# Yotsuei/ClearConverse

Hardware: AMD Instinct MI355X
Metric: xRT (audio-sec/wall-sec) end-to-end, 30 s 16 kHz clips (higher is better)
Workload: dtype bf16

## Files before the change

### clearconverse_amd/_lib.py

```python
from __future__ import annotations

import ctypes as C
import os
from pathlib import Path
from typing import Optional

_PKG = Path(__file__).resolve().parent
LIB_PATH = _PKG / "libccx.so"


class CcxError(RuntimeError):
    pass


class WhisperDims(C.Structure):
    _fields_ = [(n, C.c_int) for n in (
        "n_mels", "n_audio_ctx", "n_audio_state", "n_audio_head", "n_audio_layer",
        "n_vocab", "n_text_ctx", "n_text_state", "n_text_head", "n_text_layer")]


class SepformerDims(C.Structure):
    _fields_ = [(n, C.c_int) for n in (
        "n_filters", "kernel", "stride", "d_model", "n_head", "d_ffn", "n_layers", "n_blocks", "segment", "n_spk")]


class DecodeRules(C.Structure):
    _fields_ = [(n, C.c_int) for n in (
        "eot", "sot", "sot_prev", "no_speech", "no_timestamps", "timestamp_begin", "blank",
        "max_initial_timestamp_index", "n_suppress")] + [("suppress", C.POINTER(C.c_int))]


class DecodeOptions(C.Structure):
    _fields_ = [("without_timestamps", C.c_int), ("suppress_blank", C.c_int), ("max_initial_timestamp_index", C.c_int),
                ("n_suppress", C.c_int), ("suppress", C.POINTER(C.c_int))]


class GemmDesc(C.Structure):
    _fields_ = [
        ("A", C.c_void_p), ("W", C.c_void_p), ("lda", C.c_int64), ("ldw", C.c_int64),
        ("M", C.c_int), ("N", C.c_int), ("K", C.c_int), ("ntaps", C.c_int), ("a_tap_stride", C.c_int64),
        ("bias", C.c_void_p), ("out", C.c_void_p), ("ldo", C.c_int64), ("resid", C.c_void_p), ("ldr", C.c_int64),
        ("resid_mod", C.c_int), ("scale", C.c_void_p), ("shift", C.c_void_p), ("slope", C.c_float),
        ("rpb_in", C.c_int), ("rpb_out", C.c_int), ("roff", C.c_int), ("rpb_valid", C.c_int),
        ("img_rows_in", C.c_int), ("img_rows_valid", C.c_int), ("img_rows_out", C.c_int),
        ("resid_bf16", C.c_void_p), ("ldrb", C.c_int64),
        ("hq", C.c_void_p), ("hk", C.c_void_p), ("hv", C.c_void_p),
        ("d_model", C.c_int), ("n_head", C.c_int), ("S", C.c_int), ("Spad", C.c_int),
        ("v_transposed", C.c_int), ("first_block", C.c_int),
        ("a_elems", C.c_int64), ("w_elems", C.c_int64), ("out_elems", C.c_int64), ("resid_elems", C.c_int64),
        ("resid_bf16_elems", C.c_int64), ("heads_elems", C.c_int64)]


class DecAttnDesc(C.Structure):
    _fields_ = [
        ("q", C.c_void_p), ("k", C.c_void_p), ("v", C.c_void_p),
        ("rows", C.c_int), ("n_seq", C.c_int), ("H", C.c_int), ("kv_T", C.c_int), ("T", C.c_int),
        ("pos", C.POINTER(C.c_int)), ("row_seq", C.POINTER(C.c_int)), ("rows_per_seq", C.c_int),
        ("nsplit", C.c_int), ("combine", C.c_int), ("lds_pad", C.c_int),
        ("x", C.c_void_p), ("pend", C.c_void_p), ("pend_n", C.c_int), ("pend_stride", C.c_int64),
        ("ln_g", C.c_void_p), ("ln_b", C.c_void_p), ("eps", C.c_float),
        ("wq_host", C.c_void_p), ("bq", C.c_void_p),
        ("out", C.c_void_p), ("part_o", C.c_void_p), ("part_ml", C.c_void_p), ("q_x_out", C.c_void_p),
        ("q_elems", C.c_int64), ("kv_elems", C.c_int64), ("out_elems", C.c_int64), ("part_o_elems", C.c_int64),
        ("part_ml_elems", C.c_int64), ("x_elems", C.c_int64), ("pend_elems", C.c_int64), ("q_x_out_elems", C.c_int64),
        ("ind", C.POINTER(C.c_uint16)), ("ind_ld", C.c_int)]


DEC_ATTN_SELF, DEC_ATTN_SPLIT, DEC_ATTN_STREAM, DEC_ATTN_PREFILL, DEC_ATTN_FUSED_Q, DEC_ATTN_TWO_LAUNCH_Q = range(6)
DEC_ATTN_STREAM_MAPPED = 7
DEC_ATTN_SELF_IND = 8


class DecLnLinearDesc(C.Structure):
    _fields_ = [
        ("M", C.c_int), ("K", C.c_int), ("F", C.c_int), ("N", C.c_int), ("epi", C.c_int), ("packed", C.c_int),
        ("x", C.c_void_p), ("ln_g", C.c_void_p), ("ln_b", C.c_void_p), ("eps", C.c_float),
        ("w1_host", C.c_void_p), ("b1", C.c_void_p), ("w_host", C.c_void_p), ("bias", C.c_void_p),
        ("out", C.c_void_p), ("x_elems", C.c_int64), ("out_elems", C.c_int64)]


class DecodeSamplingOptions(C.Structure):
    _fields_ = [("top_k", C.c_int), ("top_p", C.c_float), ("min_p", C.c_float)]


class DecSeqState(C.Structure):
    _fields_ = [(n, C.c_int) for n in ("pos", "prompt_len", "n_gen", "done", "last_tok", "pen_tok", "last_ts_tok", "n_tokens")] + [
        ("sum_logprob", C.c_float), ("no_speech_prob", C.c_float)]


class DecSelectDesc(C.Structure):
    _fields_ = [
        ("logits", C.c_void_p), ("ld", C.c_int64), ("n_vocab", C.c_int), ("B", C.c_int),
        ("rules", C.POINTER(DecodeRules)), ("state", C.POINTER(DecSeqState)),
        ("prompt", C.POINTER(C.c_int)), ("max_prompt", C.c_int), ("sample_len", C.c_int),
        ("gen", C.POINTER(C.c_int)), ("cur_tok", C.POINTER(C.c_int)), ("pos", C.POINTER(C.c_int)), ("n_done", C.POINTER(C.c_int)),
        ("tok_emb", C.c_void_p), ("pos_emb", C.c_void_p), ("x", C.c_void_p), ("D", C.c_int),
        ("sample", C.c_int), ("temperature", C.c_float), ("seed", C.c_uint64), ("row0", C.c_int),
        ("logits_elems", C.c_int64), ("tok_emb_elems", C.c_int64), ("pos_emb_elems", C.c_int64), ("x_elems", C.c_int64),
        ("stream_ids", C.POINTER(C.c_int)), ("opts", C.POINTER(DecodeOptions)),
        ("sampling", C.POINTER(DecodeSamplingOptions)), ("cut_out", C.POINTER(C.c_float)), ("kept_out", C.POINTER(C.c_int)),
        ("kept_mass_out", C.POINTER(C.c_float))]


class DecBeamDesc(C.Structure):
    _fields_ = [
        ("logits", C.c_void_p), ("ld", C.c_int64), ("n_vocab", C.c_int),
        ("G", C.c_int), ("beam_size", C.c_int), ("max_candidates", C.c_int),
        ("rules", C.POINTER(DecodeRules)), ("state", C.POINTER(DecSeqState)), ("sample_len", C.c_int),
        ("hist", C.POINTER(C.c_int)), ("cur_tok", C.POINTER(C.c_int)), ("pos", C.POINTER(C.c_int)), ("n_done", C.POINTER(C.c_int)),
        ("tok_emb", C.c_void_p), ("pos_emb", C.c_void_p), ("x", C.c_void_p), ("D", C.c_int),
        ("ind", C.POINTER(C.c_uint16)), ("ind_ld", C.c_int),
        ("fin_tok", C.POINTER(C.c_int)), ("fin_score", C.POINTER(C.c_float)), ("fin_n", C.POINTER(C.c_int)),
        ("fin_count", C.POINTER(C.c_int)),
        ("cand_id", C.POINTER(C.c_int)), ("cand_lp", C.POINTER(C.c_float)), ("tok_out", C.POINTER(C.c_int)),
        ("parent_out", C.POINTER(C.c_int)),
        ("logits_elems", C.c_int64), ("tok_emb_elems", C.c_int64), ("pos_emb_elems", C.c_int64), ("x_elems", C.c_int64),
        ("opts", C.POINTER(DecodeOptions))]


class DecodeHistoryOptions(C.Structure):
    _fields_ = [("repetition_penalty", C.c_float), ("no_repeat_ngram_size", C.c_int)]


# ... 141 lines not shown
_ip = C.POINTER(C.c_int)
_i32p = C.POINTER(C.c_int32)
_i64p = C.POINTER(C.c_int64)
_fp = C.POINTER(C.c_float)

PROTOTYPES = {
    "ccx_version": (C.c_char_p, []),
    "ccx_ctx_create": (_i, [_i, C.POINTER(_vp)]),
    "ccx_ctx_destroy": (None, [_vp]),
    "ccx_last_error": (C.c_char_p, [_vp]),
    "ccx_prof_enable": (_i, [_vp, _i]),
    "ccx_prof_count": (_i, [_vp]),
    "ccx_prof_get": (_i, [_vp, _i, C.c_char_p, _i, C.POINTER(C.c_double), C.POINTER(C.c_double), _fp]),
    "ccx_gemm_bf16": (_i, [_vp, _i, _vp, _i64, _vp, _i64, _vp, _vp, _i64, _vp, _i64, _i, _i, _i, _vp]),
    "ccx_gemm_bf16_desc": (_i, [_vp, _i, C.POINTER(GemmDesc), _vp]),
    "ccx_layernorm": (_i, [_vp, _vp, _vp, _vp, _vp, _vp, _i, _i, _f, _vp]),
    "ccx_gather_rows": (_i, [_vp, _vp, _vp, _i, _i, _vp, _i64, _vp]),
    "ccx_peak_normalize": (_i, [_vp, _vp, _vp, _i64, _vp, _i, _f, _vp]),
    "ccx_row_variance": (_i, [_vp, _vp, _i64, _vp, _i, _vp, _vp]),
    "ccx_cross_attention_xa": (_i, [_vp, _vp, _vp, _vp, _vp, _vp, _vp, _i, _i, _i, _i, _i, _vp, _vp]),
    "ccx_cosine_rows": (_i, [_vp, _vp, _vp, _i, _i, _i, _vp, _vp]),
    "ccx_speaker_profiles": (_i, [_vp, _vp, _vp, _vp, _i, _i, _i, _i, _vp, _vp]),
    "ccx_resample_sinc": (_i, [_vp, _vp, _i64, _vp, _i, _i, _i, _i, _vp, _vp, _i64, _vp, _i, _vp]),
    "ccx_enc_attention": (_i, [_vp, _vp, _vp, _vp, _vp, _i, _i, _i, _i, _vp]),
    "ccx_whisper_create": (_i, [_vp, C.POINTER(WhisperDims), _i, C.POINTER(_vp)]),
    "ccx_whisper_destroy": (None, [_vp]),
    "ccx_whisper_set_tensor": (_i, [_vp, C.c_char_p, _vp, _i, _i, _i64p]),
    "ccx_whisper_set_max_audio": (_i, [_vp, C.c_double]),
    "ccx_whisper_share_encoder_scratch": (_i, [_vp, _vp]),
    "ccx_whisper_finalize": (_i, [_vp]),
    "ccx_whisper_set_rules": (_i, [_vp, C.POINTER(DecodeRules)]),
    "ccx_whisper_logmel": (_i, [_vp, _vp, _i64, _ip, _ip, _i, _vp, _vp]),
    "ccx_whisper_logmel_ex": (_i, [_vp, _vp, _i64, _ip, _ip, _ip, _i, _vp, _vp]),
    "ccx_decode_options_default": (None, [C.POINTER(DecodeOptions)]),
    "ccx_whisper_set_decode_options": (_i, [_vp, C.POINTER(DecodeOptions)]),
    "ccx_whisper_graph_count": (_i, [_vp, _i]),
    "ccx_decode_history_options_default": (None, [C.POINTER(DecodeHistoryOptions)]),
    "ccx_whisper_set_history_options": (_i, [_vp, C.POINTER(DecodeHistoryOptions)]),
    "ccx_whisper_history_graph_count": (_i, [_vp]),
    "ccx_dec_history_step": (_i, [_vp, C.POINTER(DecHistoryDesc), _vp]),
    "ccx_decode_bias_options_default": (None, [C.POINTER(DecodeBiasOptions)]),
    "ccx_whisper_set_bias_options": (_i, [_vp, C.POINTER(DecodeBiasOptions)]),
    "ccx_whisper_bias_graph_count": (_i, [_vp]),
    "ccx_dec_bias_step": (_i, [_vp, C.POINTER(DecBiasDesc), _vp]),
    "ccx_decode_sampling_options_default": (None, [C.POINTER(DecodeSamplingOptions)]),
    "ccx_whisper_set_sampling_options": (_i, [_vp, C.POINTER(DecodeSamplingOptions)]),
    "ccx_whisper_sampling_graph_count": (_i, [_vp]),
    "ccx_whisper_set_mel": (_i, [_vp, _vp, _i, _vp]),
    "ccx_whisper_encode": (_i, [_vp, _i, _vp, _vp]),
    "ccx_whisper_decoder_logits": (_i, [_vp, _i32p, _i, _i, _vp, _vp]),
    "ccx_whisper_decode_greedy": (_i, [_vp, _i32p, _i32p, _i, _i, _i, _i32p, _i32p, _fp, _fp, _vp]),
    "ccx_dec_attention_desc": (_i, [_vp, _i, C.POINTER(DecAttnDesc), _vp]),
    "ccx_dec_ln_linear": (_i, [_vp, C.POINTER(DecLnLinearDesc), _vp]),
    "ccx_dec_select_step": (_i, [_vp, C.POINTER(DecSelectDesc), _vp]),
    "ccx_dec_beam_step": (_i, [_vp, C.POINTER(DecBeamDesc), _vp]),
    "ccx_whisper_decode_beam": (_i, [_vp, _i32p, _i32p, _i, _i, _i32p, _i, _i, _i, _i, _i32p, _i32p, _fp, _i32p, _fp,
                                     C.POINTER(BeamTrace), _vp]),
    "ccx_dec_token_probs": (_i, [_vp, C.POINTER(DecTokenProbsDesc), _vp]),
    "ccx_dec_pick_probs": (_i, [_vp, C.POINTER(DecPickProbsDesc), _vp]),
    "ccx_align_op": (_i, [_vp, _i, C.POINTER(AlignDesc), _vp]),
    "ccx_whisper_align": (_i, [_vp, _i32p, _i32p, _i, _i, _i32p, _i32p, _i, _i, _vp, _vp, _i32p, _vp]),
    "ccx_whisper_align_probs": (_i, [_vp, _i32p, _i32p, _i, _i, _i32p, _i32p, _i, _i, _vp, _vp, _i32p, _i, _fp, _vp]),
    "ccx_whisper_last_cross_path": (_i, [_vp]),
    "ccx_whisper_set_sot_tail": (_i, [_vp, _i]),
    "ccx_whisper_set_prefix_len": (_i, [_vp, _i]),
    "ccx_whisper_detect_language": (_i, [_vp, _i, _i, _i, _i32p, _fp, _vp]),
    "ccx_whisper_prepare_lanes": (_i, [_vp, _vp]),
    "ccx_whisper_trace_lanes": (_i, [_vp, C.c_char_p, _i]),
    "ccx_whisper_decode": (_i, [_vp, _i32p, _i32p, _i, _i, _i, _f, C.c_uint64, _i32p, _i32p, _fp, _fp, _vp]),
    "ccx_whisper_decode_rows": (_i, [_vp, _i32p, _i32p, _i, _i, _i32p, _i, _i32p, _i, _f, C.c_uint64, _i32p, _i32p, _fp, _fp, _vp]),
    "ccx_sepformer_create": (_i, [_vp, C.POINTER(SepformerDims), _i, _i, C.POINTER(_vp)]),
    "ccx_sepformer_destroy": (None, [_vp]),
    "ccx_sepformer_set_tensor": (_i, [_vp, C.c_char_p, _vp, _i64]),
    "ccx_sepformer_finalize": (_i, [_vp]),
    "ccx_sepformer_separate": (_i, [_vp, _vp, _i64, _ip, _i, _vp, _vp]),
    "ccx_sep_op": (_i, [_vp, _i, C.POINTER(SepDesc), _vp]),
    "ccx_speaker_create": (_i, [_vp, _i, _i, _i, _i, _i64, C.POINTER(_vp)]),
    "ccx_speaker_destroy": (None, [_vp]),
    "ccx_speaker_set_tensor": (_i, [_vp, C.c_char_p, _vp, _i64]),
    "ccx_speaker_finalize": (_i, [_vp]),
    "ccx_speaker_embed": (_i, [_vp, _vp, _i64p, _ip, _i, _vp, _i64p, _ip, _vp, _vp]),
    "ccx_speaker_segment": (_i, [_vp, _vp, _i64p, _ip, _i, _vp, _i64, _ip, _vp]),
    "ccx_speaker_op": (_i, [_vp, _i, C.POINTER(SpeakerDesc), _vp]),
    "ccx_ecapa_create": (_i, [_vp, _i, _i64, C.POINTER(_vp)]),
    "ccx_ecapa_destroy": (None, [_vp]),
    "ccx_ecapa_set_tensor": (_i, [_vp, C.c_char_p, _vp, _i64]),
    "ccx_ecapa_finalize": (_i, [_vp]),
    "ccx_ecapa_embed": (_i, [_vp, _vp, _i64p, _ip, _i, _vp, _vp]),
    "ccx_ecapa_op": (_i, [_vp, _i, C.POINTER(EcapaDesc), _vp]),
    "ccx_resnet_create": (_i, [_vp, _i, _i64, _i, C.POINTER(_vp)]),
    "ccx_resnet_destroy": (None, [_vp]),
    "ccx_resnet_set_tensor": (_i, [_vp, C.c_char_p, _vp, _i64]),
    "ccx_resnet_finalize": (_i, [_vp]),
    "ccx_resnet_embed": (_i, [_vp, _vp, _i64, _i, _i, _vp, _i, _ip, _i, _vp, _vp]),
    "ccx_resnet_op": (_i, [_vp, _i, C.POINTER(ResnetDesc), _vp]),
    "ccx_specgate_create": (_i, [_vp, _i64, _i, _i, C.POINTER(_vp)]),
    "ccx_specgate_destroy": (None, [_vp]),
    "ccx_specgate_reduce": (_i, [_vp, _vp, _i64, _ip, _i, _f, _vp, _vp]),
    "ccx_specgate_reduce_long": (_i, [_vp, _vp, _i64, _f, _vp, _vp]),
    "ccx_specgate_set_clip_noise": (_i, [_vp, _i]),
    "ccx_specgate_opts_default": (None, [C.POINTER(SpecgateOpts)]),
    "ccx_specgate_reduce_ex": (_i, [_vp, C.POINTER(SpecgateOpts), _vp, _i64, _ip, _i, _vp, _vp]),
    "ccx_specgate_reduce_long_ex": (_i, [_vp, C.POINTER(SpecgateOpts), _vp, _i64, _vp, _vp]),
    "ccx_specgate_time_smooth": (_i, [_vp, _vp, _vp, _ip, _i, _i64, _f, _vp]),
}

# ... 80 lines not shown
```

### clearconverse_amd/csrc/cross_x.h

```cpp
#pragma once
#include "ccx_common.h"

struct XsParams {
  const float* q;
  const float* x; const float* pend; int pend_n; long pend_stride;
  float* x_out;
  const float* ln_g; const float* ln_b; float eps;
  const bf16_t* Wq;
  const float* bq;
  const bf16_t* xb; const float2* ln_stats; const float* ln_s;
  const bf16_t* WkT;
  bf16_t* xq;
  float* part_o;
  float* part_ml;
  const bf16_t* X;
  long x_seq_stride;
  const int* row_seq;
  int rows_per_seq;
  const bf16_t* Wv;
  const float* bv;
  bf16_t* out;
  int rows, H, S, D;
  float scale_log2e;
  int lds_pad;
  int full_lines;
};

int ccx_xs_full_lines_switch();

#define XS_SPLIT 2
static inline size_t ccx_xs_part_o_elems(size_t rows, int H, int D) { return rows * XS_SPLIT * (size_t)H * D; }
static inline size_t ccx_xs_part_ml_elems(size_t rows) { return rows * XS_SPLIT * 16 * 2; }
int ccx_launch_xs_cross_attention(ccx_ctx* ctx, const XsParams& p, hipStream_t stream);
bool ccx_xs_supported(int D, int H);
```

### clearconverse_amd/csrc/cross_x.hip

```cpp
#include "cross_x.h"
#include "dec_ln.h"

namespace {

typedef __attribute__((ext_vector_type(4))) uint32_t u32x4;
typedef __attribute__((ext_vector_type(2))) uint32_t u32x2;

__device__ __forceinline__ bf16x8 pack8(const float4 a, const float4 b) {
  const u32x4 v = {pack_bf16x2(a.x, a.y), pack_bf16x2(a.z, a.w), pack_bf16x2(b.x, b.y), pack_bf16x2(b.z, b.w)};
  return __builtin_bit_cast(bf16x8, v);
}

}

template <int D>
__global__ __launch_bounds__(256) void dec_xq_expand_kernel(XsParams p) {
  constexpr int FW = D / 4, NMT = FW / 16;
  const int h = blockIdx.x, r0 = blockIdx.y * 16;
  const int wave = threadIdx.x >> 6, lane = threadIdx.x & 63, n = lane & 15, g = lane >> 4;
  int row = r0 + n;
  const bool live = row < p.rows;
  if (!live) row = p.rows - 1;
  bf16x8 qb[2];
#pragma unroll
  for (int ks = 0; ks < 2; ks++) {
    const float4* src = (const float4*)(p.q + (long)row * D + h * 64 + ks * 32 + g * 8);
    qb[ks] = pack8(src[0], src[1]);
  }
  const bf16_t* wbase = p.WkT + ((long)h * D + wave * FW + n) * 64 + g * 8;
  bf16_t* dst = p.xq + ((long)row * p.H + h) * D + wave * FW + g * 4;
#pragma unroll
  for (int mt = 0; mt < NMT; mt++) {
    const bf16x8 a0 = *(const bf16x8*)(wbase + (long)mt * 16 * 64);
    const bf16x8 a1 = *(const bf16x8*)(wbase + (long)mt * 16 * 64 + 32);
    f32x4 c = {0.f, 0.f, 0.f, 0.f};
    c = __builtin_amdgcn_mfma_f32_16x16x32_bf16(a0, qb[0], c, 0, 0, 0);
    c = __builtin_amdgcn_mfma_f32_16x16x32_bf16(a1, qb[1], c, 0, 0, 0);
    if (live) *(u32x2*)(dst + mt * 16) = (u32x2){pack_bf16x2(c[0], c[1]), pack_bf16x2(c[2], c[3])};
  }
}

__device__ __forceinline__ float xs_wave_sum(float v) { return wave_reduce_sum(v); }

template <int D>
__global__ __launch_bounds__(256) void dec_xq_fused_kernel(XsParams p) {
  constexpr int NKS = D / 32, FW = D / 4, NMT = FW / 16, RSX = 2 * D + 16, RSQ = 2 * 64 + 16, NV = D / 4, NI = (NV + 63) / 64;
  __shared__ __attribute__((aligned(16))) char xn_s[16 * RSX];
  __shared__ __attribute__((aligned(16))) char q_s[16 * RSQ];
  const int h = blockIdx.x, r0 = blockIdx.y * 16;
  const int wave = threadIdx.x >> 6, lane = threadIdx.x & 63, n = lane & 15, g = lane >> 4;
  bf16x8 wq[NKS];
  {
    const bf16_t* wsrc = p.Wq + (long)(h * 64 + wave * 16 + n) * D + g * 8;
#pragma unroll
    for (int ks = 0; ks < NKS; ks++) wq[ks] = *(const bf16x8*)(wsrc + ks * 32);
  }
  {
    float4 gg[NI], bb[NI];
#pragma unroll
    for (int i = 0; i < NI; i++) {
      const int idx = lane + 64 * i, ic = idx < NV ? idx : 0;
      gg[i] = ((const float4*)p.ln_g)[ic];
      bb[i] = ((const float4*)p.ln_b)[ic];
    }
#pragma unroll
    for (int rr = 0; rr < 4; rr++) {
      const int lr = wave * 4 + rr;
      int m = r0 + lr;
      const bool live = m < p.rows;
      if (!live) m = p.rows - 1;
      float4 v[NI];
      float sm = 0.f;
#pragma unroll
      for (int i = 0; i < NI; i++) {
        const int idx = lane + 64 * i, ic = idx < NV ? idx : 0;
        float4 a = ((const float4*)(p.x + (long)m * D))[ic];
        float4 q[4];
#pragma unroll
        for (int s2 = 0; s2 < 4; s2++) q[s2] = ((const float4*)(p.pend + (long)(s2 < p.pend_n ? s2 : 0) * p.pend_stride + (long)m * D))[ic];
#pragma unroll
        for (int s2 = 0; s2 < 4; s2++) a = ln_add_pend(a, s2 < p.pend_n ? 1.f : 0.f, q[s2]);
        if (idx >= NV) a = make_float4(0.f, 0.f, 0.f, 0.f);
        v[i] = a;
        if (p.x_out && h == 0 && live && idx < NV) ((float4*)(p.x_out + (long)m * D))[idx] = a;
        sm += ln_sum4(a);
      }
      const float mean = xs_wave_sum(sm) / (float)D;
      float sq = 0.f;
#pragma unroll
      for (int i = 0; i < NI; i++) {
        const float t = ln_sq4(v[i], mean);
        sq += (lane + 64 * i < NV) ? t : 0.f;
      }
      const float rstd = rsqrtf(xs_wave_sum(sq) / (float)D + p.eps);
#pragma unroll
      for (int i = 0; i < NI; i++) {
        const int idx = lane + 64 * i;
        if (idx < NV) *(uint2*)(xn_s + lr * RSX + idx * 8) = ln_pack4(v[i], mean, rstd, gg[i], bb[i]);
      }
    }
  }
  __syncthreads();
  f32x4 ca = {0.f, 0.f, 0.f, 0.f}, cb = {0.f, 0.f, 0.f, 0.f};
  {
    const char* xsrc = xn_s + n * RSX + g * 16;
#pragma unroll
    for (int ks = 0; ks < NKS; ks++) {
      const bf16x8 b = *(const bf16x8*)(xsrc + ks * 64);
      if (ks & 1) cb = __builtin_amdgcn_mfma_f32_16x16x32_bf16(wq[ks], b, cb, 0, 0, 0);
      else ca = __builtin_amdgcn_mfma_f32_16x16x32_bf16(wq[ks], b, ca, 0, 0, 0);
    }
  }
  const bf16_t* wbase = p.WkT + ((long)h * D + wave * FW + n) * 64 + g * 8;
  bf16x8 wk[NMT][2];
#pragma unroll
  for (int mt = 0; mt < NMT; mt++) {
    wk[mt][0] = *(const bf16x8*)(wbase + (long)mt * 16 * 64);
    wk[mt][1] = *(const bf16x8*)(wbase + (long)mt * 16 * 64 + 32);
  }
  {
    const float4 bias = *(const float4*)(p.bq + h * 64 + wave * 16 + g * 4);
    const float v0 = ca[0] + cb[0] + bias.x, v1 = ca[1] + cb[1] + bias.y, v2 = ca[2] + cb[2] + bias.z, v3 = ca[3] + cb[3] + bias.w;
    *(u32x2*)(q_s + n * RSQ + (wave * 16 + g * 4) * 2) = (u32x2){pack_bf16x2(v0, v1), pack_bf16x2(v2, v3)};
  }
  __syncthreads();
  const bf16x8 qb0 = *(const bf16x8*)(q_s + n * RSQ + g * 16), qb1 = *(const bf16x8*)(q_s + n * RSQ + 64 + g * 16);
  const int row = r0 + n;
  bf16_t* dst = p.xq + ((long)(row < p.rows ? row : p.rows - 1) * p.H + h) * D + wave * FW + g * 4;
#pragma unroll
  for (int mt = 0; mt < NMT; mt++) {
    f32x4 c = {0.f, 0.f, 0.f, 0.f};
    c = __builtin_amdgcn_mfma_f32_16x16x32_bf16(wk[mt][0], qb0, c, 0, 0, 0);
    c = __builtin_amdgcn_mfma_f32_16x16x32_bf16(wk[mt][1], qb1, c, 0, 0, 0);
    if (row < p.rows) *(u32x2*)(dst + mt * 16) = (u32x2){pack_bf16x2(c[0], c[1]), pack_bf16x2(c[2], c[3])};
  }
}

template <int D>
__global__ __launch_bounds__(256) void dec_xq_lnfree_kernel(XsParams p) {
  constexpr int NKS = D / 32, FW = D / 4, NMT = FW / 16, RSQ = 2 * 64 + 16;
  __shared__ __attribute__((aligned(16))) char q_s[16 * RSQ];
  __shared__ float2 st_s[16];
  const int h = blockIdx.x, r0 = blockIdx.y * 16;
  const int wave = threadIdx.x >> 6, lane = threadIdx.x & 63, n = lane & 15, g = lane >> 4;
  int row = r0 + n;
  const bool live = row < p.rows;
  if (!live) row = p.rows - 1;
  bf16x8 wq[NKS], xb[NKS];
  {
    const bf16_t* wsrc = p.Wq + (long)(h * 64 + wave * 16 + n) * D + g * 8;
    const bf16_t* xsrc = p.xb + (long)row * D + g * 8;
#pragma unroll
    for (int ks = 0; ks < NKS; ks++) wq[ks] = *(const bf16x8*)(wsrc + ks * 32);
#pragma unroll
    for (int ks = 0; ks < NKS; ks++) xb[ks] = *(const bf16x8*)(xsrc + ks * 32);
  }
  if (threadIdx.x < 64) {
    const int r = threadIdx.x >> 2, qt = threadIdx.x & 3;
    int m = r0 + r;
    m = m < p.rows ? m : p.rows - 1;
    constexpr int T4 = (D / 16) / 4;
    const float2* sp = p.ln_stats + (long)m * (D / 16) + qt * T4;
    float s1 = 0.f, s2 = 0.f;
#pragma unroll
    for (int i = 0; i < T4; i++) {
      const float2 v = sp[i];
      s1 += v.x; s2 += v.y;
    }
    s1 += dpp_mov<CCX_DPP_QUAD_XOR1>(s1); s2 += dpp_mov<CCX_DPP_QUAD_XOR1>(s2);
    s1 += dpp_mov<CCX_DPP_QUAD_XOR2>(s1); s2 += dpp_mov<CCX_DPP_QUAD_XOR2>(s2);
    const float mean = s1 / (float)D;
    const float var = fmaf(-mean, mean, s2 / (float)D);
    if (qt == 0) st_s[r] = make_float2(mean, rsqrtf(fmaxf(var, 0.f) + p.eps));
  }
  const bf16_t* wbase = p.WkT + ((long)h * D + wave * FW + n) * 64 + g * 8;
  bf16x8 wk[NMT][2];
#pragma unroll
  for (int mt = 0; mt < NMT; mt++) {
    wk[mt][0] = *(const bf16x8*)(wbase + (long)mt * 16 * 64);
    wk[mt][1] = *(const bf16x8*)(wbase + (long)mt * 16 * 64 + 32);
  }
  const float4 cc = *(const float4*)(p.bq + h * 64 + wave * 16 + g * 4);
  const float4 ss = *(const float4*)(p.ln_s + h * 64 + wave * 16 + g * 4);
  f32x4 ca = {0.f, 0.f, 0.f, 0.f}, cb = {0.f, 0.f, 0.f, 0.f};
#pragma unroll
  for (int ks = 0; ks < NKS; ks++) {
    if (ks & 1) cb = __builtin_amdgcn_mfma_f32_16x16x32_bf16(wq[ks], xb[ks], cb, 0, 0, 0);
    else ca = __builtin_amdgcn_mfma_f32_16x16x32_bf16(wq[ks], xb[ks], ca, 0, 0, 0);
  }
  __syncthreads();
  {
    const float2 ms = st_s[n];
    const float v0 = fmaf(ms.y, fmaf(-ms.x, ss.x, ca[0] + cb[0]), cc.x), v1 = fmaf(ms.y, fmaf(-ms.x, ss.y, ca[1] + cb[1]), cc.y);
    const float v2 = fmaf(ms.y, fmaf(-ms.x, ss.z, ca[2] + cb[2]), cc.z), v3 = fmaf(ms.y, fmaf(-ms.x, ss.w, ca[3] + cb[3]), cc.w);
    *(u32x2*)(q_s + n * RSQ + (wave * 16 + g * 4) * 2) = (u32x2){pack_bf16x2(v0, v1), pack_bf16x2(v2, v3)};
  }
  __syncthreads();
  const bf16x8 qb0 = *(const bf16x8*)(q_s + n * RSQ + g * 16), qb1 = *(const bf16x8*)(q_s + n * RSQ + 64 + g * 16);
  bf16_t* dst = p.xq + ((long)row * p.H + h) * D + wave * FW + g * 4;
#pragma unroll
  for (int mt = 0; mt < NMT; mt++) {
    f32x4 c = {0.f, 0.f, 0.f, 0.f};
    c = __builtin_amdgcn_mfma_f32_16x16x32_bf16(wk[mt][0], qb0, c, 0, 0, 0);
    c = __builtin_amdgcn_mfma_f32_16x16x32_bf16(wk[mt][1], qb1, c, 0, 0, 0);
    if (live) *(u32x2*)(dst + mt * 16) = (u32x2){pack_bf16x2(c[0], c[1]), pack_bf16x2(c[2], c[3])};
  }
}

template <int D>
__global__ __launch_bounds__(256) void dec_xv_project_kernel(XsParams p) {
  constexpr int NKS = D / 32, RSB = 2 * D + 16;
  __shared__ __attribute__((aligned(16))) char ctx_s[16 * RSB];
  const int h = blockIdx.x, r0 = blockIdx.y * 16;
  const int wave = threadIdx.x >> 6, lane = threadIdx.x & 63, n = lane & 15, g = lane >> 4;
  const int o0 = h * 64 + wave * 16;
  const bf16_t* wsrc = p.Wv + (long)(o0 + n) * D + g * 8;
  constexpr int CH = NKS % 6 == 0 ? 6 : 4;
  static_assert(NKS % CH == 0, "D must be a multiple of 128");
  bf16x8 a[CH];
#pragma unroll
  for (int k = 0; k < CH; k++) a[k] = *(const bf16x8*)(wsrc + k * 32);
  {
    const int rr = threadIdx.x >> 4, c = threadIdx.x & 15;
    int row = r0 + rr;
    if (row >= p.rows) row = p.rows - 1;
    float m[XS_SPLIT], l[XS_SPLIT], wgt[XS_SPLIT];
    float mx = -INFINITY;
#pragma unroll
    for (int s2 = 0; s2 < XS_SPLIT; s2++) {
      const float2 ml = *(const float2*)(p.part_ml + (((long)row * XS_SPLIT + s2) * 16 + h) * 2);
      m[s2] = ml.x; l[s2] = ml.y;
      mx = fmaxf(mx, ml.x);
    }
    float den = 0.f;
#pragma unroll
    for (int s2 = 0; s2 < XS_SPLIT; s2++) {
      wgt[s2] = __builtin_amdgcn_exp2f(m[s2] - mx);
      den = fmaf(l[s2], wgt[s2], den);
    }
    const float inv = 1.f / den;
#pragma unroll
    for (int s2 = 0; s2 < XS_SPLIT; s2++) wgt[s2] *= inv;
    const float* src = p.part_o + (((long)row * XS_SPLIT) * p.H + h) * D;
    const long sstride = (long)p.H * D;
#pragma unroll
    for (int k = 0; k < D / 64; k++) {
      const int f = (c + 16 * k) * 4;
      float4 v = make_float4(0.f, 0.f, 0.f, 0.f);
#pragma unroll
      for (int s2 = 0; s2 < XS_SPLIT; s2++) {
        const float4 o = *(const float4*)(src + s2 * sstride + f);
        v.x = fmaf(o.x, wgt[s2], v.x); v.y = fmaf(o.y, wgt[s2], v.y); v.z = fmaf(o.z, wgt[s2], v.z); v.w = fmaf(o.w, wgt[s2], v.w);
      }
      *(u32x2*)(ctx_s + rr * RSB + f * 2) = (u32x2){pack_bf16x2(v.x, v.y), pack_bf16x2(v.z, v.w)};
    }
  }
  __syncthreads();
  const char* csrc = ctx_s + n * RSB + g * 16;
  f32x4 ca = {0.f, 0.f, 0.f, 0.f}, cb = {0.f, 0.f, 0.f, 0.f};
#pragma unroll
  for (int c0 = 0; c0 < NKS; c0 += CH) {
    bf16x8 an[CH];
    if (c0 + CH < NKS) {
#pragma unroll
      for (int k = 0; k < CH; k++) an[k] = *(const bf16x8*)(wsrc + (c0 + CH + k) * 32);
    }
#pragma unroll
    for (int k = 0; k < CH; k++) {
      const bf16x8 b = *(const bf16x8*)(csrc + (c0 + k) * 64);
      if (k & 1) cb = __builtin_amdgcn_mfma_f32_16x16x32_bf16(a[k], b, cb, 0, 0, 0);
      else ca = __builtin_amdgcn_mfma_f32_16x16x32_bf16(a[k], b, ca, 0, 0, 0);
    }
    if (c0 + CH < NKS) {
#pragma unroll
      for (int k = 0; k < CH; k++) a[k] = an[k];
    }
  }
  const int row = r0 + n;
  if (row < p.rows) {
    const float4 bias = *(const float4*)(p.bv + o0 + g * 4);
    const float v0 = ca[0] + cb[0] + bias.x, v1 = ca[1] + cb[1] + bias.y, v2 = ca[2] + cb[2] + bias.z, v3 = ca[3] + cb[3] + bias.w;
    *(u32x2*)(p.out + (long)row * D + o0 + g * 4) = (u32x2){pack_bf16x2(v0, v1), pack_bf16x2(v2, v3)};
  }
}

namespace {
#ifndef CCX_XS_FULL_NT
#define CCX_XS_FULL_NT 1
#endif
template <int D, int RB = 1, int FL = 0>
struct XsGeom {
  static constexpr int FW = D / 4;
  static constexpr int NKS = FW / 32;
  static constexpr int NMT = FW / 16;
  static constexpr int PF = 4;
  static constexpr int RS = 2 * FW + 32;
  static constexpr int STRIP = 16 * RS;
  static constexpr int NSTRIP = FL ? 2 : 1;
  static constexpr int S_OFF = 4 * NSTRIP * STRIP;
  static constexpr int LDS = S_OFF + 2 * RB * 4 * 1024;
  static_assert(!FL || (D / 2) % 128 == 0, "full lines: a wave's quarter of a key row must be whole 128-byte lines");
  static_assert(!FL || PF % 2 == 0, "full lines: the strip of a tile is the parity of its slot");
};
template <int D> constexpr bool xs_full_lines_ok = (D / 2) % 128 == 0;
}

template <int D, int RB, int FL>
__global__ __launch_bounds__(256, RB == 1 ? 2 : 1) void dec_xs_stream_kernel(XsParams p) {
  using G = XsGeom<D, RB, FL>;
  constexpr int FW = G::FW, NKS = G::NKS, NMT = G::NMT, PF = G::PF, RS = G::RS, STRIP = G::STRIP;
  constexpr bool FULL = FL != 0, NT_HINT = CCX_XS_FULL_NT != 0;
  extern __shared__ __attribute__((aligned(16))) char xs_smem[];
  const int unit = blockIdx.x / XS_SPLIT, sp = blockIdx.x % XS_SPLIT;
  int row0, nrow;
  if (RB == 1) { row0 = unit; nrow = 1; }
  else {
    const int groups = (p.rows_per_seq + RB - 1) / RB;
    const int s_idx = unit / groups, gi = unit - s_idx * groups;
    row0 = s_idx * p.rows_per_seq + gi * RB;
    nrow = p.rows_per_seq - gi * RB < RB ? p.rows_per_seq - gi * RB : RB;
  }
  const int seq = p.row_seq ? p.row_seq[row0] : row0;
  const int wave = threadIdx.x >> 6, lane = threadIdx.x & 63, r = lane & 15, g = lane >> 4;
  const int H = p.H, S = p.S;
  char* strip = xs_smem + wave * (G::NSTRIP * STRIP);
  char* sbuf = xs_smem + G::S_OFF;

  const int lk = FULL ? lane >> 3 : r, lc = FULL ? lane & 7 : g;
  const bf16_t* Xp = p.X + (long)seq * p.x_seq_stride + wave * FW + lc * 8;
  const int NTall = (S + 15) >> 4;
  const int T0 = NTall * sp / XS_SPLIT, NT = NTall * (sp + 1) / XS_SPLIT;

  bf16x8 img[PF][NKS];
  auto load_tile = [&](bf16x8 (&X)[NKS], int t) {
    int key = t * 16 + lk;
// ... 187 lines not shown
  CCX_REQUIRE(ctx, p.rows_per_seq <= 1 || p.row_seq != nullptr, "xs cross attention: rows_per_seq = %d needs row_seq", p.rows_per_seq);
  const bool multi = p.rows_per_seq > 1;
  CCX_REQUIRE(ctx, p.rows_per_seq <= 1 || p.rows % p.rows_per_seq == 0, "xs cross attention: %d rows are not a multiple of %d rows per sequence", p.rows, p.rows_per_seq);
  const dim3 small_grid(p.H, ccx_cdiv(p.rows, 16));
  const double wbytes = (double)p.H * 64 * D * 2;
  if (p.xb) {
    ccx_prof_scope ps(ctx, stream, D == 768 ? "dec_xq_lnfree_kernel<768>" : "dec_xq_lnfree_kernel", 2.0 * p.rows * D * (double)D * 2,
                      2.0 * wbytes + (double)p.rows * D * 2 + (double)p.rows * p.H * D * 2);
    hipLaunchKernelGGL(dec_xq_lnfree_kernel<D>, small_grid, dim3(256), 0, stream, p);
  } else if (p.x) {
    ccx_prof_scope ps(ctx, stream, D == 768 ? "dec_xq_fused_kernel<768>" : "dec_xq_fused_kernel", 2.0 * p.rows * D * (double)D * 2,
                      2.0 * wbytes + (double)p.rows * D * 4 * (1 + p.pend_n) + (double)p.rows * p.H * D * 2);
    hipLaunchKernelGGL(dec_xq_fused_kernel<D>, small_grid, dim3(256), 0, stream, p);
  } else {
    ccx_prof_scope ps(ctx, stream, D == 768 ? "dec_xq_expand_kernel<768>" : "dec_xq_expand_kernel", 2.0 * p.rows * p.H * 64 * D, wbytes + (double)p.rows * D * 4 + (double)p.rows * p.H * D * 2);
    hipLaunchKernelGGL(dec_xq_expand_kernel<D>, small_grid, dim3(256), 0, stream, p);
  }
  CCX_CHECK_LAUNCH(ctx);
  {
    ccx_prof_scope ps(ctx, stream, D == 768 ? (multi ? "dec_xs_stream_kernel<768,4>" : "dec_xs_stream_kernel<768,1>") : "dec_xs_stream_kernel", 4.0 * p.rows * 16 * (double)p.S * D,
                      (double)p.rows * ((double)p.S * D * 2 + p.H * D * 2.0 + XS_SPLIT * p.H * D * 4.0));
    int rc;
    if constexpr (xs_full_lines_ok<D>) {
      rc = p.full_lines ? launch_xs_stream<D, 1>(ctx, p, stream) : launch_xs_stream<D, 0>(ctx, p, stream);
    } else {
      rc = launch_xs_stream<D, 0>(ctx, p, stream);
    }
    if (rc != CCX_OK) return rc;
  }
  CCX_CHECK_LAUNCH(ctx);
  {
    ccx_prof_scope ps(ctx, stream, D == 768 ? "dec_xv_project_kernel<768>" : "dec_xv_project_kernel", 2.0 * p.rows * p.H * 64 * D, wbytes + (double)p.rows * p.H * D * 2 + (double)p.rows * D * 2);
    hipLaunchKernelGGL(dec_xv_project_kernel<D>, small_grid, dim3(256), 0, stream, p);
  }
  CCX_CHECK_LAUNCH(ctx);
  return CCX_OK;
}

}

int ccx_xs_full_lines_switch() {
  const char* e = getenv("CCX_XS_FULL_LINES");
  return !e || atoi(e) != 0;
}

bool ccx_xs_supported(int D, int H) { return H >= 1 && H <= 16 && H * 64 == D && (D == 128 || D == 256 || D == 384 || D == 512 || D == 768); }

int ccx_launch_xs_cross_attention(ccx_ctx* ctx, const XsParams& p, hipStream_t stream) {
  CCX_REQUIRE(ctx, ccx_xs_supported(p.D, p.H), "xs cross attention: width %d with %d heads is not instantiated", p.D, p.H);
  CCX_REQUIRE(ctx, p.rows >= 1 && p.S >= 16 && (p.q || p.x || p.xb) && p.WkT && p.xq && p.X && p.Wv && p.bv && p.out, "xs cross attention: bad arguments");
  CCX_REQUIRE(ctx, !p.xb || (p.ln_stats && p.ln_s && p.Wq && p.bq), "xs cross attention: bad LayerNorm-free query arguments");
  CCX_REQUIRE(ctx, !p.x || (p.pend && p.ln_g && p.ln_b && p.Wq && p.bq && p.pend_n >= 0 && p.pend_n <= 4 && p.x_out != p.x), "xs cross attention: bad fused-query arguments");
  CCX_REQUIRE(ctx, p.part_o && p.part_ml, "xs cross attention: partial buffers missing");
  switch (p.D) {
    case 128: return launch_xs<128>(ctx, p, stream);
    case 256: return launch_xs<256>(ctx, p, stream);
    case 384: return launch_xs<384>(ctx, p, stream);
    case 512: return launch_xs<512>(ctx, p, stream);
    default: return launch_xs<768>(ctx, p, stream);
  }
}

namespace {
__global__ void xs_bf16_to_f32_kernel(const bf16_t* __restrict__ in, float* __restrict__ out, long n) {
  const long i = (long)blockIdx.x * 256 + threadIdx.x;
  if (i < n) out[i] = bf16_to_f32(in[i]);
}
}

extern "C" int ccx_cross_attention_xa(ccx_ctx* ctx, const float* q_dev, const float* wk_host, const float* wv_host, const float* bv_host,
                                      const uint16_t* xa_dev, const int* row_seq_host, int rows_per_seq, int rows, int n_seq, int n_head,
                                      int n_ctx, float* out_dev, void* stream_) {
  if (!ctx) return CCX_ERR_ARG;
  hipStream_t stream = (hipStream_t)stream_;
  const int H = n_head, D = 64 * n_head, S = n_ctx;
  CCX_REQUIRE(ctx, ccx_xs_supported(D, H), "cross_attention_xa: %d heads (width %d) not instantiated", H, D);
  CCX_REQUIRE(ctx, q_dev && wk_host && wv_host && bv_host && xa_dev && out_dev && rows >= 1 && n_seq >= 1 && S >= 16, "cross_attention_xa: bad arguments");
  if (row_seq_host)
    for (int i = 0; i < rows; i++) CCX_REQUIRE(ctx, row_seq_host[i] >= 0 && row_seq_host[i] < n_seq, "cross_attention_xa: row_seq[%d] out of range", i);
  else CCX_REQUIRE(ctx, rows <= n_seq, "cross_attention_xa: more rows than sequences without a row map");
  if (rows_per_seq > 1) {
    CCX_REQUIRE(ctx, row_seq_host && rows % rows_per_seq == 0, "cross_attention_xa: rows_per_seq needs a row map and a multiple of it in rows");
    for (int i = 0; i < rows; i++)
      CCX_REQUIRE(ctx, row_seq_host[i] == row_seq_host[i - i % rows_per_seq], "cross_attention_xa: row %d is not in its group's sequence", i);
  }
  std::vector<bf16_t> wkt((size_t)D * D), wv((size_t)D * D);
  for (int hh = 0; hh < H; hh++)
    for (int f = 0; f < D; f++)
      for (int dd = 0; dd < 64; dd++) wkt[((size_t)hh * D + f) * 64 + dd] = ccx_host_f32_to_bf16(wk_host[(size_t)(hh * 64 + dd) * D + f]);
  for (size_t i = 0; i < wv.size(); i++) wv[i] = ccx_host_f32_to_bf16(wv_host[i]);
  bf16_t *d_wkt = nullptr, *d_wv = nullptr, *d_xq = nullptr, *d_out = nullptr;
  float *d_bv = nullptr, *d_po = nullptr, *d_pml = nullptr;
  int* d_rs = nullptr;
  auto cleanup = [&]() { hipFree(d_wkt); hipFree(d_wv); hipFree(d_xq); hipFree(d_out); hipFree(d_bv); hipFree(d_rs); hipFree(d_po); hipFree(d_pml); };
#define XS_TRY(expr) do { hipError_t e_ = (expr); if (e_ != hipSuccess) { cleanup(); return ccx_fail(ctx, CCX_ERR_HIP, "%s failed: %s", #expr, hipGetErrorString(e_)); } } while (0)
  XS_TRY(hipMalloc(&d_wkt, wkt.size() * 2)); XS_TRY(hipMalloc(&d_wv, wv.size() * 2)); XS_TRY(hipMalloc(&d_bv, (size_t)D * 4));
  XS_TRY(hipMalloc(&d_xq, (size_t)rows * H * D * 2)); XS_TRY(hipMalloc(&d_out, (size_t)rows * D * 2));
  XS_TRY(hipMalloc(&d_po, ccx_xs_part_o_elems(rows, H, D) * 4)); XS_TRY(hipMalloc(&d_pml, ccx_xs_part_ml_elems(rows) * 4));
  XS_TRY(hipMemcpy(d_wkt, wkt.data(), wkt.size() * 2, hipMemcpyHostToDevice));
  XS_TRY(hipMemcpy(d_wv, wv.data(), wv.size() * 2, hipMemcpyHostToDevice));
  XS_TRY(hipMemcpy(d_bv, bv_host, (size_t)D * 4, hipMemcpyHostToDevice));
  if (row_seq_host) {
    XS_TRY(hipMalloc(&d_rs, (size_t)rows * 4));
    XS_TRY(hipMemcpy(d_rs, row_seq_host, (size_t)rows * 4, hipMemcpyHostToDevice));
  }
  XsParams p;
  memset(&p, 0, sizeof(p));
  p.q = q_dev; p.WkT = d_wkt; p.xq = d_xq; p.X = xa_dev; p.x_seq_stride = (long)S * D; p.row_seq = d_rs; p.Wv = d_wv; p.bv = d_bv; p.out = d_out; p.part_o = d_po; p.part_ml = d_pml;
  p.rows = rows; p.H = H; p.S = S; p.D = D; p.scale_log2e = 0.125f * 1.4426950408889634f;
  p.rows_per_seq = rows_per_seq > 1 ? rows_per_seq : 0;
  p.full_lines = ccx_xs_full_lines_switch();
  int rc =ccx_launch_xs_cross_attention(ctx, p, stream);
  if (rc == CCX_OK) {
    const long n = (long)rows * D;
    hipLaunchKernelGGL(xs_bf16_to_f32_kernel, dim3((unsigned)((n + 255) / 256)), dim3(256), 0, stream, d_out, out_dev, n);
    XS_TRY(hipStreamSynchronize(stream));
  }
  cleanup();
#undef XS_TRY
  return rc;
}
```

### clearconverse_amd/csrc/dec_ops.hip

```cpp
#include "../../include/ccx.h"
#include "ccx_common.h"
#include "decoder.h"
#include "op_scratch.h"

static_assert(sizeof(ccx_dec_seq_state) == sizeof(DecSeqState), "ccx_dec_seq_state mirrors DecSeqState field for field");

namespace {

__global__ void dec_ops_bf16_to_f32_kernel(const bf16_t* __restrict__ in, float* __restrict__ out, long n) {
  const long i = (long)blockIdx.x * 256 + threadIdx.x;
  if (i < n) out[i] = bf16_to_f32(in[i]);
}

}

extern "C" int ccx_dec_attention_desc(ccx_ctx* ctx, int form, const ccx_dec_attn_desc* d, void* stream_) {
  if (!ctx) return CCX_ERR_ARG;
  hipStream_t stream = (hipStream_t)stream_;
  CCX_REQUIRE(ctx, d != nullptr, "ccx_dec_attention_desc: desc is NULL");
  CCX_REQUIRE(ctx, (form >= CCX_DEC_ATTN_SELF && form <= CCX_DEC_ATTN_TWO_LAUNCH_Q) || form == CCX_DEC_ATTN_STREAM_MAPPED || form == CCX_DEC_ATTN_SELF_IND,
              "ccx_dec_attention_desc: unknown form %d", form);
  const bool is_ind = form == CCX_DEC_ATTN_SELF_IND;
  const bool is_self = form == CCX_DEC_ATTN_SELF || is_ind, is_split = form == CCX_DEC_ATTN_SPLIT, is_mapped = form == CCX_DEC_ATTN_STREAM_MAPPED,
             is_stream = form == CCX_DEC_ATTN_STREAM || is_mapped;
  const bool is_prefill = form == CCX_DEC_ATTN_PREFILL, with_q = form == CCX_DEC_ATTN_FUSED_Q || form == CCX_DEC_ATTN_TWO_LAUNCH_Q;
  const bool partials = is_split || with_q;
  const bool final_out = is_self || is_stream || is_prefill || (is_split && d->combine);
  const int rows = d->rows, H = d->H, n_seq = d->n_seq, kv_T = d->kv_T;
  CCX_REQUIRE(ctx, rows >= 1 && rows <= 65536 && n_seq >= 1 && n_seq <= 65536 && H >= 1 && H <= 64 && kv_T >= 1 && kv_T <= (1 << 20),
              "ccx_dec_attention_desc: rows=%d, n_seq=%d, H=%d or kv_T=%d out of range", rows, n_seq, H, kv_T);
  CCX_REQUIRE(ctx, d->k && d->v && ccx_aligned16(d->k) && ccx_aligned16(d->v), "ccx_dec_attention_desc: k / v null or not 16-byte aligned");
  const int64_t kv_need = (int64_t)n_seq * H * kv_T * 64;
  CCX_REQUIRE(ctx, kv_need <= d->kv_elems, "ccx_dec_attention_desc: k / v are read up to element %ld, kv_elems=%ld", (long)kv_need, (long)d->kv_elems);
  if (is_ind) {
    CCX_REQUIRE(ctx, d->row_seq == nullptr, "ccx_dec_attention_desc: row_seq is not taken by form %d (the rows read through ind)", form);
  } else if (is_self || is_split || is_prefill || is_mapped) {
    if (d->row_seq)
      for (int i = 0; i < rows; i++)
        CCX_REQUIRE(ctx, d->row_seq[i] >= 0 && d->row_seq[i] < n_seq, "ccx_dec_attention_desc: row_seq[%d] = %d out of range [0, %d)", i, d->row_seq[i], n_seq);
    else CCX_REQUIRE(ctx, rows <= n_seq, "ccx_dec_attention_desc: row_seq is NULL with more rows (%d) than sequences (%d)", rows, n_seq);
  } else {
    CCX_REQUIRE(ctx, d->row_seq == nullptr, "ccx_dec_attention_desc: row_seq is not taken by form %d (row r reads sequence r)", form);
    CCX_REQUIRE(ctx, rows <= n_seq, "ccx_dec_attention_desc: more rows (%d) than sequences (%d)", rows, n_seq);
  }
  if (is_prefill) {
    const int P = d->rows_per_seq;
    CCX_REQUIRE(ctx, P >= 2 && P <= 4096, "ccx_dec_attention_desc: rows_per_seq = %d, the prefill form needs >= 2", P);
    CCX_REQUIRE(ctx, d->row_seq && rows % P == 0, "ccx_dec_attention_desc: rows_per_seq needs row_seq and a multiple of it in rows");
    for (int i = 0; i < rows; i++) {
      CCX_REQUIRE(ctx, d->row_seq[i] == d->row_seq[i - i % P], "ccx_dec_attention_desc: row %d is not in its group's sequence (row_seq)", i);
      CCX_REQUIRE(ctx, d->row_seq[i] == i / P, "ccx_dec_attention_desc: row_seq[%d] = %d, the prefill form needs group g on sequence g", i, d->row_seq[i]);
    }
  } else CCX_REQUIRE(ctx, d->rows_per_seq <= 1, "ccx_dec_attention_desc: rows_per_seq = %d is taken by the prefill form only", d->rows_per_seq);
  if (is_self) {
    CCX_REQUIRE(ctx, d->pos != nullptr, "ccx_dec_attention_desc: pos is NULL");
// ... 148 lines not shown
  bf16_t *d_xn = nullptr, *d_ffn = nullptr, *d_w1 = nullptr, *d_w = nullptr, *d_g16 = nullptr, *d_ck = nullptr, *d_cv = nullptr;
  float* d_pend = nullptr; int* d_pos = nullptr;
  DO_HIP(sc.alloc(&d_xn, Mp * K));
  DO_HIP(hipMemsetAsync(d_xn, 0xFF, Mp * K * 2, stream));
  DO_HIP(sc.alloc(&d_pend, (size_t)M * K));
  DO_HIP(hipMemsetAsync(d_pend, 0, (size_t)M * K * 4, stream));
  DO_HIP(hipMemsetAsync(d->out, 0xFF, (size_t)n_out * 4, stream));
  {
    const std::vector<bf16_t> pw = pack_mfma_rows(d->w_host, N, Kin, 32);
    DO_HIP(sc.upload(&d_w, pw.data(), pw.size()));
  }
  int rc = ccx_launch_dec_resolve_ln(ctx, (const float*)d->x, d_pend, 0, (long)M * K, (const float*)d->ln_g, (const float*)d->ln_b, d_xn, nullptr, M, K,
                                     d->eps, stream, nullptr, packed);
  const bf16_t* act = d_xn;
  if (rc == CCX_OK && F > 0) {
    const std::vector<bf16_t> pw1 = pack_mfma_rows(d->w1_host, F, K, 32);
    DO_HIP(sc.upload(&d_w1, pw1.data(), pw1.size()));
    DO_HIP(sc.alloc(&d_ffn, Mp * F));
    DO_HIP(hipMemsetAsync(d_ffn, 0xFF, Mp * F * 2, stream));
    DecLinearParams lp;
    memset(&lp, 0, sizeof(lp));
    lp.M = M; lp.N = F; lp.K = K; lp.W = d_w1; lp.ldw = K; lp.bias = (const float*)d->b1; lp.act = d_xn; lp.lda = K; lp.act_packed = packed;
    lp.out = d_ffn; lp.ldo = F; lp.out_packed = packed;
    rc = ccx_launch_dec_linear(ctx, ACT_BF16, DEPI_BF16_GELU, lp, stream);
    act = d_ffn;
  }
  if (rc == CCX_OK) {
    DecLinearParams lp;
    memset(&lp, 0, sizeof(lp));
    lp.M = M; lp.N = N; lp.K = Kin; lp.W = d_w; lp.ldw = Kin; lp.bias = (const float*)d->bias; lp.act = act; lp.lda = Kin; lp.act_packed = packed;
    lp.out = d->out; lp.ldo = N; lp.pend_stride = (long)M * N;
    if (epi == CCX_DEC_EPI_SELF_QKV) {
      const std::vector<int> pos((size_t)M, 0);
      DO_HIP(sc.upload(&d_pos, pos.data(), pos.size()));
      DO_HIP(sc.alloc(&d_ck, (size_t)M * K)); DO_HIP(sc.alloc(&d_cv, (size_t)M * K));
      DO_HIP(hipMemsetAsync(d_ck, 0xFF, (size_t)M * K * 2, stream)); DO_HIP(hipMemsetAsync(d_cv, 0xFF, (size_t)M * K * 2, stream));
      lp.ldo = K; lp.cache_k = d_ck; lp.cache_v = d_cv; lp.cache_T = 1; lp.pos = d_pos;
    } else if (epi == CCX_DEC_EPI_GELU) {
      DO_HIP(sc.alloc(&d_g16, Mp * N));
      DO_HIP(hipMemsetAsync(d_g16, 0xFF, Mp * N * 2, stream));
      lp.out = d_g16; lp.out_packed = packed;
    }
    rc = ccx_launch_dec_linear(ctx, ACT_BF16, depi, lp, stream);
    if (rc == CCX_OK && epi == CCX_DEC_EPI_SELF_QKV) {
      const long n = (long)M * K;
      hipLaunchKernelGGL(dec_ops_rows_to_f32_kernel, dim3((unsigned)((n + 255) / 256)), dim3(256), 0, stream, d_ck, (float*)d->out + n, M, K, 0);
      hipLaunchKernelGGL(dec_ops_rows_to_f32_kernel, dim3((unsigned)((n + 255) / 256)), dim3(256), 0, stream, d_cv, (float*)d->out + 2 * n, M, K, 0);
      DO_HIP(hipGetLastError());
    } else if (rc == CCX_OK && epi == CCX_DEC_EPI_GELU) {
      const long n = (long)M * N;
      hipLaunchKernelGGL(dec_ops_rows_to_f32_kernel, dim3((unsigned)((n + 255) / 256)), dim3(256), 0, stream, d_g16, (float*)d->out, M, N, packed);
      DO_HIP(hipGetLastError());
    }
  }
  DO_HIP(hipStreamSynchronize(stream));
  return rc;
}

extern "C" int ccx_dec_select_step(ccx_ctx* ctx, const ccx_dec_select_desc* d, void* stream_) {
  if (!ctx) return CCX_ERR_ARG;
  hipStream_t stream = (hipStream_t)stream_;
  CCX_REQUIRE(ctx, d != nullptr, "ccx_dec_select_step: desc is NULL");
  const int V = d->n_vocab, B = d->B, D = d->D;
  CCX_REQUIRE(ctx, B >= 1 && B <= 65536, "ccx_dec_select_step: B = %d out of range", B);
  CCX_REQUIRE(ctx, V >= 4 && V % 4 == 0 && V <= 13 * 4096, "ccx_dec_select_step: n_vocab = %d must be a multiple of 4 and <= 53248", V);
  CCX_REQUIRE(ctx, d->ld >= V && d->ld % 4 == 0, "ccx_dec_select_step: ld = %ld must be >= n_vocab and a multiple of 4", (long)d->ld);
  CCX_REQUIRE(ctx, d->logits && ccx_aligned16(d->logits), "ccx_dec_select_step: logits null or not 16-byte aligned");
  CCX_REQUIRE(ctx, (int64_t)(B - 1) * d->ld + V <= d->logits_elems, "ccx_dec_select_step: logits are read up to element %ld, logits_elems=%ld",
              (long)((int64_t)(B - 1) * d->ld + V), (long)d->logits_elems);
  CCX_REQUIRE(ctx, d->rules && d->state && d->gen && d->cur_tok && d->pos && d->n_done, "ccx_dec_select_step: rules, state, gen, cur_tok, pos or n_done is NULL");
  const ccx_decode_rules& r = *d->rules;
  std::vector<unsigned char> mask;
  CCX_TRY(ccx_build_suppress_mask(ctx, "ccx_dec_select_step", &r, V, mask));
  int max_init_ts = r.max_initial_timestamp_index, no_rules = 0, sup_blank = 1;
  if (const ccx_decode_options* o = d->opts) {
    CCX_TRY(ccx_build_options_mask(ctx, "ccx_dec_select_step", &r, o, V, mask));
    no_rules = o->without_timestamps; sup_blank = o->suppress_blank;
    if (o->max_initial_timestamp_index != -2) max_init_ts = o->max_initial_timestamp_index;
  }
  CCX_REQUIRE(ctx, r.no_speech >= 0 && r.timestamp_begin >= 0 && r.blank >= 0, "ccx_dec_select_step: rules.no_speech, timestamp_begin or blank negative");
  CCX_REQUIRE(ctx, d->sample_len >= 1 && d->sample_len <= (1 << 20), "ccx_dec_select_step: sample_len = %d out of range", d->sample_len);
  CCX_REQUIRE(ctx, d->max_prompt >= 0 && (d->max_prompt == 0 || d->prompt), "ccx_dec_select_step: prompt is NULL with max_prompt = %d", d->max_prompt);
  CCX_REQUIRE(ctx, D >= 4 && D % 4 == 0 && D <= 4096, "ccx_dec_select_step: D = %d must be a multiple of 4 in [4, 4096]", D);
  CCX_REQUIRE(ctx, d->tok_emb && d->pos_emb && d->x && ccx_aligned16(d->tok_emb) && ccx_aligned16(d->pos_emb) && ccx_aligned16(d->x),
              "ccx_dec_select_step: tok_emb, pos_emb or x null or not 16-byte aligned");
  CCX_REQUIRE(ctx, (int64_t)V * D <= d->tok_emb_elems, "ccx_dec_select_step: tok_emb is read up to element %ld, tok_emb_elems=%ld", (long)V * D, (long)d->tok_emb_elems);
  CCX_REQUIRE(ctx, (int64_t)B * D <= d->x_elems, "ccx_dec_select_step: x is written up to element %ld, x_elems=%ld", (long)B * D, (long)d->x_elems);
  const int64_t pos_rows = d->pos_emb_elems / D;
  CCX_REQUIRE(ctx, d->sample == 0 || d->sample == 1, "ccx_dec_select_step: sample = %d must be 0 or 1", d->sample);
  CCX_REQUIRE(ctx, d->sample || d->temperature == 0.f, "ccx_dec_select_step: temperature %g needs sample = 1", (double)d->temperature);
  CCX_REQUIRE(ctx, d->temperature >= 0.f && d->row0 >= 0, "ccx_dec_select_step: temperature or row0 negative");
  ccx_decode_sampling_options trunc{0, 1.0f, 0.0f};
  if (d->sampling) {
    CCX_REQUIRE(ctx, d->sample == 1, "ccx_dec_select_step: sampling options need sample = 1");
    trunc = *d->sampling;
    CCX_TRY(ccx_check_sampling_options(ctx, "ccx_dec_select_step", &trunc));
  }
  CCX_REQUIRE(ctx, d->sampling || (!d->cut_out && !d->kept_out && !d->kept_mass_out), "ccx_dec_select_step: cut_out, kept_out and kept_mass_out need sampling options");
  if (d->stream_ids)
    for (int b = 0; b < B; b++) CCX_REQUIRE(ctx, d->stream_ids[b] >= 0, "ccx_dec_select_step: stream_ids[%d] = %d is negative", b, d->stream_ids[b]);
  for (int b = 0; b < B; b++) {
    const ccx_dec_seq_state& s = d->state[b];
    CCX_REQUIRE(ctx, s.n_gen >= 0 && s.n_gen <= d->sample_len, "ccx_dec_select_step: state[%d].n_gen = %d out of range [0, sample_len = %d]", b, s.n_gen, d->sample_len);
    CCX_REQUIRE(ctx, s.pos >= 0 && s.pos + 1 < pos_rows, "ccx_dec_select_step: state[%d].pos = %d, pos + 1 must be a row of pos_emb (%ld rows)", b, s.pos, (long)pos_rows);
    CCX_REQUIRE(ctx, s.prompt_len >= 0 && s.prompt_len <= d->max_prompt, "ccx_dec_select_step: state[%d].prompt_len = %d out of range [0, max_prompt = %d]", b, s.prompt_len, d->max_prompt);
    CCX_REQUIRE(ctx, s.done == 0 || s.done == 1, "ccx_dec_select_step: state[%d].done = %d must be 0 or 1", b, s.done);
// ... 188 lines not shown
```

### clearconverse_amd/csrc/decoder.h

```cpp
#pragma once
#include <cstring>
#include <vector>
#include "../../include/ccx.h"
#include "ccx_common.h"

enum { ACT_LN = 0, ACT_BF16 = 1, ACT_COMBINE = 2 };
enum { DEPI_BF16_GELU = 1, DEPI_PARTIAL = 2, DEPI_F32 = 3, DEPI_SELF_QKV = 4, DEPI_RESOLVE = 5 };

struct DecLinearParams {
  int M, N, K;
  const bf16_t* W; long ldw;
  const float* bias;
  const float* x;
  const float* pend; int pend_n; long pend_stride;
  float* x_out;
  const float* ln_g; const float* ln_b; float eps;
  float* ln_mean_out;
  const bf16_t* act; long lda;
  const float* part_o; const float* part_ml; int nsplit;
  float* xres; bf16_t* xb; float2* st_out; const float* shift; float shift_c;
  void* out; long ldo;
  bf16_t* cache_k; bf16_t* cache_v; int cache_T; const int* pos; const int* row_seq;
  int act_packed, out_packed;
};
int ccx_launch_dec_linear(ccx_ctx* ctx, int act, int epi, const DecLinearParams& p, hipStream_t stream);
int ccx_dec_linear_ksplit(int K, int epi);
int ccx_launch_dec_resolve_ln(ccx_ctx* ctx, const float* x, const float* pend, int pend_n, long pend_stride, const float* g,
                              const float* b, bf16_t* out, float* x_out, int M, int K, float eps, hipStream_t stream,
                              float* mean_out = nullptr, int out_packed = 0);

__host__ __device__ __forceinline__ long dec_frag_off(int m, int k, int ksteps) {
  return (((long)(m >> 4) * ksteps + (k >> 5)) * 64 + (((k >> 3) & 3) * 16 + (m & 15))) * 8 + (k & 7);
}
int ccx_dec_packed_act_switch();

struct DecAttnParams {
  const float* q;
  const bf16_t* k;
  const bf16_t* v;
  int H, kv_T;
  const int* pos;
  int T;
  float scale_log2e;
  bf16_t* out_bf16;
  float* part_o;
  float* part_ml;
  int lds_pad;
  int stream_mode;
  const int* row_seq; int rows_per_seq;
  const float* qx; const float* q_pend; int q_pend_n; long q_pend_stride; float* q_x_out;
  const float* q_ln_g; const float* q_ln_b; float q_eps;
  const bf16_t* q_W; const float* q_bias; int q_K;
  int kv_map;
  const unsigned short* ind; int ind_ld;
};
int ccx_launch_dec_attention(ccx_ctx* ctx, const DecAttnParams& p, int B, int nsplit, bool final_out, hipStream_t stream);
int ccx_launch_dec_cross_fused_q(ccx_ctx* ctx, const DecAttnParams& p, int B, int nsplit, hipStream_t stream);

struct DecSeqState {
  int pos, prompt_len, n_gen, done;
  int last_tok, pen_tok, last_ts_tok, n_tokens;
  float sum_logprob, no_speech_prob;
};

struct DecSelectParams {
  const float* logits; long ld_logits; int n_vocab;
  DecSeqState* state;
  const int* prompt; int max_prompt;
  int* cur_tok; int* pos;
  int* gen; int sample_len;
  int* n_done;
  const unsigned char* suppress_mask;
  int eot, blank, no_speech, timestamp_begin, max_initial_ts;
  const float* tok_emb; const float* pos_emb; float* x; int D;
  const unsigned* sample_cfg; int row0;
  int sample;
  const int* stream_id;
  int no_rules, suppress_blank;
  int trunc;
  float* cut_out; int* kept_out; float* kept_mass_out;
};
int ccx_launch_dec_select(ccx_ctx* ctx, const DecSelectParams& p, int B, hipStream_t stream);

constexpr int kBeamMax = 8;
constexpr int kBeamCandMax = 16;
struct DecBeamParams {
  DecSelectParams sel;
  int beam, max_cand;
  int* cand_id; float* cand_lp;
  unsigned short* ind; int ind_ld;
  int row0;
  int* fin_tok; float* fin_score; int* fin_n; int* fin_count;
  int* step_tok; int* step_parent;
  int* tr_cand_id; float* tr_cand_lp; int* tr_tok; int* tr_parent; float* tr_score; int tr_rows;
};
int ccx_launch_dec_beam(ccx_ctx* ctx, const DecBeamParams& p, int n_windows, hipStream_t stream);

constexpr int kDecHistoryMax = 2048;
struct DecHistoryParams {
  float* logits; long ld;
  const DecSeqState* state;
  const int* gen; int sample_len;
  int text_end;
  float penalty; int ngram;
};
int ccx_launch_dec_history(ccx_ctx* ctx, const DecHistoryParams& p, int rows, hipStream_t stream);

// ... 114 lines not shown
```

### clearconverse_amd/csrc/decoder.hip

```cpp
#include <string>
#include "decoder.h"

__global__ void dec_embed_kernel(const float* __restrict__ tok_emb, const float* __restrict__ pos_emb,
                                 const int* __restrict__ cur_tok, const int* __restrict__ pos, float* __restrict__ x,
                                 int D) {
  const int b = blockIdx.x;
  const float4* te = (const float4*)(tok_emb + (long)cur_tok[b] * D);
  const float4* pe = (const float4*)(pos_emb + (long)pos[b] * D);
  float4* xo = (float4*)(x + (long)b * D);
  for (int i = threadIdx.x; i < D / 4; i += blockDim.x) {
    const float4 a = te[i], c = pe[i];
    xo[i] = make_float4(a.x + c.x, a.y + c.y, a.z + c.z, a.w + c.w);
  }
}

#include "dec_ln.h"

__device__ __forceinline__ float centre_shift(float mean, float rstd) { return fabsf(mean) * rstd > 1.f ? mean : 0.f; }

__device__ __forceinline__ uint4 combine_partials(const float* part_o, const float* part_ml, int nsplit, int mh, int c) {
  const float2* ml = (const float2*)(part_ml + ((long)mh * nsplit) * 2);
  const float* ob = part_o + ((long)mh * nsplit) * 64 + 8 * c;
  float2 mlv[8];
  float4 oa[8], oc[8];
// ... 200 lines not shown
    }
    __syncthreads();
  }

  f32x4 acc[NT][MT];
#pragma unroll
  for (int i = 0; i < NT; i++)
#pragma unroll
    for (int j = 0; j < MT; j++) acc[i][j] = (f32x4){0.f, 0.f, 0.f, 0.f};
#pragma unroll
  for (int k = 0; k < KMAX; k++) {
    if (k < nks) {
      if (!BF16IN) {
#pragma unroll
        for (int j = 0; j < MT; j++)
          af[j][k] = *(const bf16x8*)(act_s + (long)(16 * j + l15) * lds_ld + 8 * h4 + 32 * (ks0 + k));
      }
#pragma unroll
      for (int i = 0; i < NT; i++)
#pragma unroll
        for (int j = 0; j < MT; j++)
          acc[i][j] = __builtin_amdgcn_mfma_f32_16x16x32_bf16(wf[i][k], af[j][k], acc[i][j], 0, 0, 0);
    }
  }

  __syncthreads();
#pragma unroll
  for (int i = 0; i < NT; i++)
#pragma unroll
    for (int j = 0; j < MT; j++) *(f32x4*)(red + (((wave * NT + i) * MT + j) * 64 + lane) * 4) = acc[i][j];
  __syncthreads();

#pragma unroll
  for (int it = 0; it < EPI_ITERS; it++) {
    const int qd = tid + NTHR * it;
    if (qd >= QUADS) break;
    const int ln = qd & 63, j = (qd >> 6) % MT, i = (qd >> 6) / MT;
    const int m = m0 + 16 * j + (ln & 15), n = n0 + 16 * i + 4 * (ln >> 4);
    if (EPI == DEPI_RESOLVE) {
      f32x4 v = *(const f32x4*)(red + (((0 * NT + i) * MT + j) * 64 + ln) * 4);
#pragma unroll
      for (int w = 1; w < NW; w++) v += *(const f32x4*)(red + (((w * NT + i) * MT + j) * 64 + ln) * 4);
      v[0] = (v[0] + bias_v[it].x) + xold_v[it].x; v[1] = (v[1] + bias_v[it].y) + xold_v[it].y;
      v[2] = (v[2] + bias_v[it].z) + xold_v[it].z; v[3] = (v[3] + bias_v[it].w) + xold_v[it].w;
      const float c0 = v[0] - shift_v[it], c1 = v[1] - shift_v[it], c2 = v[2] - shift_v[it], c3 = v[3] - shift_v[it];
      float s1 = (c0 + c1) + (c2 + c3);
      float s2 = fmaf(c3, c3, fmaf(c2, c2, fmaf(c1, c1, c0 * c0)));
      s1 += lane_xor16(s1); s2 += lane_xor16(s2);
      s1 += lane_xor32(s1); s2 += lane_xor32(s2);
      if (m < p.M && n < p.N) {
        *(float4*)(p.xres + (long)m * p.N + n) = make_float4(v[0], v[1], v[2], v[3]);
        uint2 pk;
        pk.x = pack_bf16x2(c0, c1); pk.y = pack_bf16x2(c2, c3);
        *(uint2*)(p.xb + (long)m * p.N + n) = pk;
        if ((ln >> 4) == 0) p.st_out[(long)m * (p.N >> 4) + (n >> 4)] = make_float2(s1, s2);
      }
      continue;
    }
    if (n >= p.N || m >= p.M) continue;
    f32x4 v = *(const f32x4*)(red + (((0 * NT + i) * MT + j) * 64 + ln) * 4);
#pragma unroll
    for (int w = 1; w < NW; w++) v += *(const f32x4*)(red + (((w * NT + i) * MT + j) * 64 + ln) * 4);
    v[0] += bias_v[it].x; v[1] += bias_v[it].y; v[2] += bias_v[it].z; v[3] += bias_v[it].w;
    const bool full = n + 3 < p.N;
    if (EPI == DEPI_BF16_GELU) {
      bf16_t* o = (bf16_t*)p.out + (BF16IN && p.out_packed ? dec_frag_off(m, n, p.N >> 5) : (long)m * p.ldo + n);
      if (full) {
        uint2 pk;
        pk.x = pack_bf16x2(gelu_erf(v[0]), gelu_erf(v[1]));
        pk.y = pack_bf16x2(gelu_erf(v[2]), gelu_erf(v[3]));
        *(uint2*)o = pk;
      } else {
        for (int c = 0; c < 4 && n + c < p.N; c++) o[c] = f32_to_bf16(gelu_erf(v[c]));
      }
    } else if (EPI == DEPI_PARTIAL || EPI == DEPI_F32) {
      float* o = (float*)p.out + (EPI == DEPI_PARTIAL ? (long)blockIdx.z * p.pend_stride : 0L) + (long)m * p.ldo + n;
      if (full) *(float4*)o = make_float4(v[0], v[1], v[2], v[3]);
      else
        for (int c = 0; c < 4 && n + c < p.N; c++) o[c] = v[c];
    } else if (EPI == DEPI_SELF_QKV) {
      const int D = p.K;
      if (n < D) {
        *(float4*)((float*)p.out + (long)m * D + n) = make_float4(v[0], v[1], v[2], v[3]);
      } else {
        const int which = (n >= 2 * D);
        const int nn = n - (which ? 2 * D : D);
        const int hh = nn >> 6, d = nn & 63;
        const int H = D >> 6;
        bf16_t* cache = which ? p.cache_v : p.cache_k;
        const int sq = p.row_seq ? p.row_seq[m] : m;
        uint2 pk;
        pk.x = pack_bf16x2(v[0], v[1]);
        pk.y = pack_bf16x2(v[2], v[3]);
        *(uint2*)(cache + (((long)sq * H + hh) * p.cache_T + pos_v[it]) * 64 + d) = pk;
      }
    }
  }
}

template <int NS>
__global__ __launch_bounds__(256) void dec_resolve_ln_kernel(const float* __restrict__ x, const float* __restrict__ pend,
                                                             int pend_n, long pend_stride, const float* __restrict__ g,
                                                             const float* __restrict__ b, bf16_t* __restrict__ out,
                                                             float* __restrict__ x_out, int M, int K, float eps,
                                                             float* __restrict__ mean_out, int out_packed) {
  const int lane = threadIdx.x & 63;
  const int m = blockIdx.x * 4 + (threadIdx.x >> 6);
// ... 84 lines not shown
    hipLaunchKernelGGL(dec_resolve_ln_kernel<5>, dim3(ccx_cdiv(M, 4)), dim3(256), 0, stream, x, pend, pend_n, pend_stride, g, b,
                       out, x_out, M, K, eps, mean_out, out_packed);
  CCX_CHECK_LAUNCH(ctx);
  return CCX_OK;
}

template <int MT, int NT, int KMAX, int ACT, int EPI>
static int launch_dec_linear_inst(ccx_ctx* ctx, const DecLinearParams& p, int ksplit, hipStream_t stream) {
  const int MROWS = 16 * MT, BN = 16 * NT;
  size_t act_bytes = ACT == ACT_BF16 ? 0 : ccx_align((size_t)MROWS * (p.K + 8) * 2, 16);
  size_t red_bytes = (size_t)4 * NT * MT * 64 * 4 * 4;
  size_t lds = act_bytes + red_bytes;
  CCX_REQUIRE(ctx, lds <= 160 * 1024, "dec_linear: LDS %zu too large", lds);
  CCX_REQUIRE(ctx, ccx_cdiv(ccx_cdiv(p.K / 32, ksplit), 4) <= KMAX, "dec_linear: K=%d / split %d exceeds the prefetch depth %d", p.K, ksplit, KMAX);
  if (EPI == DEPI_RESOLVE) CCX_REQUIRE(ctx, p.xres && p.xb && p.st_out && ksplit == 1 && p.N % BN == 0, "dec_linear: bad resolve arguments (N=%d, %d columns per block)", p.N, BN);
  static ccx_lds_optin optin;
  if (lds > 64 * 1024) CCX_HIP(ctx, optin.ensure(ctx->device, (const void*)dec_linear_kernel<MT, NT, KMAX, ACT, EPI>));
  dim3 grid(ccx_cdiv(p.N, BN), ccx_cdiv(p.M, MROWS), ksplit);
  {
    static const std::string label = "dec_linear_kernel<" + std::to_string(MT) + ", " + std::to_string(NT) + ", " + std::to_string(KMAX) +
                                     ", " + std::to_string(ACT) + ", " + std::to_string(EPI) + ">";
    ccx_prof_scope ps(ctx, stream, label.c_str(), 2.0 * p.M * (double)p.N * p.K,
                      2.0 * (double)p.N * p.K + 2.0 * p.M * ((double)p.K + p.N));
    hipLaunchKernelGGL((dec_linear_kernel<MT, NT, KMAX, ACT, EPI>), grid, dim3(256), lds, stream, p);
  }
  CCX_CHECK_LAUNCH(ctx);
  return CCX_OK;
}

template <int NT, int ACT, int EPI>
static int launch_dec_linear_mt(ccx_ctx* ctx, const DecLinearParams& p, int ksplit, hipStream_t stream) {
  const int M = p.M;
  const int need = ccx_cdiv(ccx_cdiv(p.K / 32, ksplit), 4);
  if (need <= 6) {
    if (M <= 16) return launch_dec_linear_inst<1, NT, 6, ACT, EPI>(ctx, p, ksplit, stream);
    if (M <= 32) return launch_dec_linear_inst<2, NT, 6, ACT, EPI>(ctx, p, ksplit, stream);
    return launch_dec_linear_inst<4, NT, 6, ACT, EPI>(ctx, p, ksplit, stream);
  }
  if (need <= 8) {
    if (M <= 16) return launch_dec_linear_inst<1, NT, 8, ACT, EPI>(ctx, p, ksplit, stream);
    if (M <= 32) return launch_dec_linear_inst<2, NT, 8, ACT, EPI>(ctx, p, ksplit, stream);
    return launch_dec_linear_inst<4, NT, 8, ACT, EPI>(ctx, p, ksplit, stream);
  }
  if (M <= 16) return launch_dec_linear_inst<1, NT, 10, ACT, EPI>(ctx, p, ksplit, stream);
  if (M <= 32) return launch_dec_linear_inst<2, NT, 10, ACT, EPI>(ctx, p, ksplit, stream);
  return launch_dec_linear_inst<4, NT, 10, ACT, EPI>(ctx, p, ksplit, stream);
}

int ccx_dec_packed_act_switch() {
  const char* e = getenv("CCX_DEC_PACKED_ACT");
  return !(e && strcmp(e, "0") == 0);
}

int ccx_dec_linear_ksplit(int K, int epi) {
  if (epi == DEPI_RESOLVE) return 1;
  int ks = ccx_cdiv(K, 1024);
  if (epi != DEPI_PARTIAL) return K <= 1280 ? 1 : ks;
  if (ks > 4) ks = ccx_cdiv(K, 1280);
  return ks < 1 ? 1 : ks;
}

int ccx_launch_dec_linear(ccx_ctx* ctx, int act, int epi, const DecLinearParams& p, hipStream_t stream) {
  CCX_REQUIRE(ctx, p.M > 0 && p.N > 0 && p.K > 0 && p.K % 32 == 0, "dec_linear: bad shape M=%d N=%d K=%d", p.M, p.N, p.K);
  CCX_REQUIRE(ctx, act == ACT_BF16 || p.K <= 1280, "dec_linear: LN/combine activation needs K <= 1280");
  CCX_REQUIRE(ctx, p.pend_n >= 0 && p.pend_n <= 4, "dec_linear: at most 4 pending slabs");
  CCX_REQUIRE(ctx, !p.act_packed || act == ACT_BF16, "dec_linear: act_packed is taken with bf16 activations only");
  CCX_REQUIRE(ctx, !p.out_packed || (act == ACT_BF16 && epi == DEPI_BF16_GELU && p.N % 32 == 0), "dec_linear: out_packed needs the GELU epilogue and N=%d a multiple of 32", p.N);
  const int ksplit = ccx_dec_linear_ksplit(p.K, epi);
  CCX_REQUIRE(ctx, epi == DEPI_PARTIAL || ksplit == 1, "dec_linear: K=%d needs a split-K (partial) epilogue", p.K);
  CCX_REQUIRE(ctx, ksplit <= 4, "dec_linear: K=%d would leave %d partial slabs (at most 4)", p.K, ksplit);
  CCX_REQUIRE(ctx, epi != DEPI_PARTIAL || p.pend_stride >= (long)p.M * p.ldo, "dec_linear: pend_stride too small");
  if (epi == DEPI_RESOLVE) {
    CCX_REQUIRE(ctx, act == ACT_BF16, "dec_linear: the resolve epilogue takes bf16 activations");
    if (p.M >= 128) return launch_dec_linear_mt<2, ACT_BF16, DEPI_RESOLVE>(ctx, p, 1, stream);
    return launch_dec_linear_mt<1, ACT_BF16, DEPI_RESOLVE>(ctx, p, 1, stream);
  }
  if (p.M >= 128 && act == ACT_BF16) {
    if (epi == DEPI_PARTIAL) return launch_dec_linear_mt<2, ACT_BF16, DEPI_PARTIAL>(ctx, p, ksplit, stream);
    if (epi == DEPI_F32) return launch_dec_linear_mt<2, ACT_BF16, DEPI_F32>(ctx, p, 1, stream);
    if (epi == DEPI_SELF_QKV) return launch_dec_linear_mt<2, ACT_BF16, DEPI_SELF_QKV>(ctx, p, 1, stream);
    if (epi == DEPI_BF16_GELU) return launch_dec_linear_mt<2, ACT_BF16, DEPI_BF16_GELU>(ctx, p, 1, stream);
  }
  if (act == ACT_LN && epi == DEPI_SELF_QKV) return launch_dec_linear_mt<1, ACT_LN, DEPI_SELF_QKV>(ctx, p, 1, stream);
  if (act == ACT_LN && epi == DEPI_F32) return launch_dec_linear_mt<1, ACT_LN, DEPI_F32>(ctx, p, 1, stream);
  if (act == ACT_LN && epi == DEPI_BF16_GELU) return launch_dec_linear_mt<1, ACT_LN, DEPI_BF16_GELU>(ctx, p, 1, stream);
  if (act == ACT_COMBINE && epi == DEPI_PARTIAL) return launch_dec_linear_mt<1, ACT_COMBINE, DEPI_PARTIAL>(ctx, p, ksplit, stream);
  if (act == ACT_BF16 && epi == DEPI_PARTIAL) return launch_dec_linear_mt<1, ACT_BF16, DEPI_PARTIAL>(ctx, p, ksplit, stream);
  if (act == ACT_BF16 && epi == DEPI_F32) return launch_dec_linear_mt<1, ACT_BF16, DEPI_F32>(ctx, p, 1, stream);
  if (act == ACT_BF16 && epi == DEPI_SELF_QKV) return launch_dec_linear_mt<1, ACT_BF16, DEPI_SELF_QKV>(ctx, p, 1, stream);
  if (act == ACT_BF16 && epi == DEPI_BF16_GELU) return launch_dec_linear_mt<1, ACT_BF16, DEPI_BF16_GELU>(ctx, p, 1, stream);
  return ccx_fail(ctx, CCX_ERR_ARG, "dec_linear: unsupported act=%d epi=%d", act, epi);
}

struct SoftState {
  float m, l, o[8];
};
__device__ __forceinline__ void soft_init(SoftState& st) {
  st.m = -1e30f; st.l = 0.f;
#pragma unroll
  for (int j = 0; j < 8; j++) st.o[j] = 0.f;
}

__device__ __forceinline__ void load_q8(float (&q)[8], const float* src) {
  const float4 a = *(const float4*)src, d = *(const float4*)(src + 4);
  q[0] = a.x; q[1] = a.y; q[2] = a.z; q[3] = a.w; q[4] = d.x; q[5] = d.y; q[6] = d.z; q[7] = d.w;
}

template <int NIT, bool NONTEMPORAL>
__device__ __forceinline__ void kv_load(bf16x8 (&kf)[NIT], bf16x8 (&vf)[NIT], const bf16_t* Kb, const bf16_t* Vb, int base, int g,
                                        int limit, int last) {
  long off[NIT];
#pragma unroll
  for (int it = 0; it < NIT; it++) {
    int key = base + it * 8 + g;
    key = key < limit ? key : last;
    off[it] = (long)key * 64;
  }
#pragma unroll
  for (int it = 0; it < NIT; it++) kf[it] = NONTEMPORAL ? __builtin_nontemporal_load((const bf16x8*)(Kb + off[it])) : *(const bf16x8*)(Kb + off[it]);
#pragma unroll
// ... 27 lines not shown
    for (int j = 0; j < 8; j++) st.o[j] = fmaf(pe, bf16_to_f32((bf16_t)vf[it][j]), st.o[j]);
  }
  st.m = mn;
}

template <bool PINNED = true>
__device__ __forceinline__ void soft_merge(SoftState& a, float bm, float bl, const float (&bo)[8]) {
  const float mx = fmaxf(a.m, bm);
  const float wa = __builtin_amdgcn_exp2f(a.m - mx), wb = __builtin_amdgcn_exp2f(bm - mx);
  a.l = a.l * wa + bl * wb;
#pragma unroll
  for (int j = 0; j < 8; j++) a.o[j] = PINNED ? fmaf(bo[j], wb, a.o[j] * wa) : a.o[j] * wa + bo[j] * wb;
  a.m = mx;
}

template <bool PINNED = true>
__device__ __forceinline__ void soft_merge_lane_groups(SoftState& st) {
  float om, ol, oo[8];
  om = dpp_mov<0x128>(st.m); ol = dpp_mov<0x128>(st.l);
#pragma unroll
  for (int j = 0; j < 8; j++) oo[j] = dpp_mov<0x128>(st.o[j]);
  soft_merge(st, om, ol, oo);
  om = lane_xor16(st.m); ol = lane_xor16(st.l);
#pragma unroll
  for (int j = 0; j < 8; j++) oo[j] = lane_xor16(st.o[j]);
  soft_merge<PINNED>(st, om, ol, oo);
  om = lane_xor32(st.m); ol = lane_xor32(st.l);
#pragma unroll
  for (int j = 0; j < 8; j++) oo[j] = lane_xor32(st.o[j]);
  soft_merge<PINNED>(st, om, ol, oo);
}

__device__ __forceinline__ void soft_store_wave(float (&sm_m)[4][8], float (&sm_l)[4][8], float (&sm_o)[4][8][8], const SoftState& st,
                                                int wave, int g, int c) {
  if (g == 0) {
    sm_m[wave][c] = st.m; sm_l[wave][c] = st.l;
#pragma unroll
    for (int j = 0; j < 8; j++) sm_o[wave][c][j] = st.o[j];
  }
}
__device__ __forceinline__ void soft_merge_waves(const float (&sm_m)[4][8], const float (&sm_l)[4][8], const float (&sm_o)[4][8][8], int d,
                                                 float& mx, float& l, float& o) {
  const int cc = d >> 3, j = d & 7;
  mx = fmaxf(fmaxf(sm_m[0][cc], sm_m[1][cc]), fmaxf(sm_m[2][cc], sm_m[3][cc]));
  l = 0.f; o = 0.f;
#pragma unroll
  for (int w = 0; w < 4; w++) {
    const float ww = __builtin_amdgcn_exp2f(sm_m[w][cc] - mx);
    l += ww * sm_l[w][cc];
    o += ww * sm_o[w][cc][j];
  }
}

template <bool FINAL, bool IND = false>
__global__ __launch_bounds__(256) void dec_attention_kernel(DecAttnParams p) {
  __shared__ float sm_m[4][8], sm_l[4][8], sm_o[4][8][8];
  const int tid = threadIdx.x, lane = tid & 63, wave = tid >> 6;
  const int bh = blockIdx.x, split = blockIdx.y;
  const int b = bh / p.H, h = bh - b * p.H;
  const int sq = p.row_seq ? p.row_seq[b] : b;
  const int g = lane >> 3, c = lane & 7;
  const int T = p.pos ? (p.pos[b] + 1) : p.T;
  const int per = (T + gridDim.y - 1) / gridDim.y;
  const int kbeg = split * per;
  const int kend = (kbeg + per < T) ? kbeg + per : T;

  const bf16_t* Kb = p.k + ((long)sq * p.H + h) * p.kv_T * 64 + 8 * c;
  const bf16_t* Vb = p.v + ((long)sq * p.H + h) * p.kv_T * 64 + 8 * c;

  SoftState st;
  soft_init(st);
  float q[8];
  load_q8(q, p.q + ((long)b * p.H + h) * 64 + 8 * c);

  for (int base = kbeg + wave * 64; base < kend; base += 256) {
    bf16x8 kf[8], vf[8];
    if (IND) {
      const unsigned short* ir = p.ind + (long)b * p.ind_ld;
      const bf16_t* K0 = p.k + 8 * c;
      const bf16_t* V0 = p.v + 8 * c;
      int key[8]; unsigned slot[8];
#pragma unroll
      for (int it = 0; it < 8; it++) {
        key[it] = base + it * 8 + g;
        key[it] = key[it] < kend ? key[it] : kend - 1;
        slot[it] = ir[key[it]];
      }
#pragma unroll
      for (int it = 0; it < 8; it++) {
        const long off = (((long)slot[it] * p.H + h) * p.kv_T + key[it]) * 64;
        kf[it] = *(const bf16x8*)(K0 + off);
        vf[it] = *(const bf16x8*)(V0 + off);
      }
      soft_update<8>(st, q, kf, vf, base, g, kend, p.scale_log2e);
      continue;
    }
#pragma unroll
    for (int it = 0; it < 8; it++) {
      int key = base + it * 8 + g;
      key = key < kend ? key : kend - 1;
      if (FINAL) {
        kf[it] = *(const bf16x8*)(Kb + (long)key * 64);
        vf[it] = *(const bf16x8*)(Vb + (long)key * 64);
      } else {
        kf[it] = __builtin_nontemporal_load((const bf16x8*)(Kb + (long)key * 64));
        vf[it] = __builtin_nontemporal_load((const bf16x8*)(Vb + (long)key * 64));
      }
    }
    soft_update<8>(st, q, kf, vf, base, g, kend, p.scale_log2e);
  }
  soft_merge_lane_groups(st);
  soft_store_wave(sm_m, sm_l, sm_o, st, wave, g, c);
  __syncthreads();
  if (tid < 64) {
    float mx, l, o;
    soft_merge_waves(sm_m, sm_l, sm_o, tid, mx, l, o);
    if (FINAL) {
      p.out_bf16[((long)b * p.H + h) * 64 + tid] = f32_to_bf16(o / l);
    } else {
      const long pbase = ((long)b * p.H + h) * gridDim.y + split;
      p.part_o[pbase * 64 + tid] = o;
      if (tid == 0) { p.part_ml[pbase * 2] = mx; p.part_ml[pbase * 2 + 1] = l; }
    }
  }
}

template <bool EARLY_V>
__global__ __launch_bounds__(256, EARLY_V ? 2 : 3) void dec_cross_fused_q_kernel(DecAttnParams p) {
  __shared__ float sm_m[4][8], sm_l[4][8], sm_o[4][8][8];
  __shared__ __attribute__((aligned(16))) bf16_t ln_row[4][776];
  __shared__ __attribute__((aligned(16))) float red[4][4][4][4];
  __shared__ __attribute__((aligned(16))) float q_s[64];
  const int tid = threadIdx.x, lane = tid & 63, wave = tid >> 6;
  const int bh = blockIdx.x, split = blockIdx.y;
  const int b = bh / p.H, h = bh - b * p.H;
  const int g = lane >> 3, c = lane & 7;
  const int T = p.T;
  const int per = (T + gridDim.y - 1) / gridDim.y;
  const int kbeg = split * per;
  const int kend = (kbeg + per < T) ? kbeg + per : T;
  const int K = p.q_K;
  const char* Ku = (const char*)(p.k + ((long)b * p.H + h) * p.kv_T * 64);
  const char* Vu = (const char*)(p.v + ((long)b * p.H + h) * p.kv_T * 64);
  bf16x8 kf[8], vf[8];
  auto load_chunk = [&](int base, bool want_k, bool want_v) {
#pragma unroll
    for (int it = 0; it < 8; it++) {
      int key = base + it * 8 + g;
      key = key < kend ? key : kend - 1;
      const unsigned off = (unsigned)(key * 64 + 8 * c) * 2u;
      if (want_k) kf[it] = __builtin_nontemporal_load((const bf16x8*)(Ku + off));
      if (want_v) vf[it] = __builtin_nontemporal_load((const bf16x8*)(Vu + off));
    }
  };

  const int nv = K >> 2;
  const long row = (long)b * K;
  float4 v[4], pq[4], gg[4], bb[4];
#pragma unroll
  for (int i = 0; i < 4; i++) {
    const int idx = lane + 64 * i;
    const int ic = idx < nv ? idx : 0;
    const unsigned o16 = (unsigned)ic * 16u;
    v[i] = *(const float4*)((const char*)(p.qx + row) + o16);
    pq[i] = *(const float4*)((const char*)(p.q_pend + row) + o16);
    gg[i] = *(const float4*)((const char*)p.q_ln_g + o16);
    bb[i] = *(const float4*)((const char*)p.q_ln_b + o16);
  }
  __builtin_amdgcn_sched_barrier(0);
  load_chunk(kbeg + wave * 64, true, EARLY_V);
  const int ksteps = K >> 5;
// ... 225 lines not shown
      load(kB, vB, base + 32 < w1 ? base + 32 : base);
#pragma unroll
      for (int r = 0; r < RB; r++) soft_update<4>(st[r], q[r], kA, vA, base, g, w1, p.scale_log2e);
#pragma unroll
      for (int it = 0; it < 4; it++) { kA[it] = kB[it]; vA[it] = vB[it]; }
    }
  }
#pragma unroll
  for (int r = 0; r < RB; r++) {
    soft_merge_lane_groups<false>(st[r]);
    soft_store_wave(sm_m[r], sm_l[r], sm_o[r], st[r], wave, g, c);
  }
  __syncthreads();
  for (int e = tid; e < RB * 64; e += 256) {
    const int r = e >> 6, d = e & 63;
    if (t0 + r >= p.rows_per_seq) continue;
    float mx, l, o;
    soft_merge_waves(sm_m[r], sm_l[r], sm_o[r], d, mx, l, o);
    p.out_bf16[((long)(sq * p.rows_per_seq + t0 + r) * p.H + h) * 64 + d] = f32_to_bf16(o / l);
  }
}

struct DecAttnKernel {
  const char* label;
  void (*fn)(DecAttnParams);
  ccx_lds_optin optin;
};

int ccx_launch_dec_attention(ccx_ctx* ctx, const DecAttnParams& p, int B, int nsplit, bool final_out,
                             hipStream_t stream) {
  CCX_REQUIRE(ctx, B > 0 && p.H > 0 && nsplit >= 1, "dec_attention: bad shape");
  CCX_REQUIRE(ctx, !final_out || nsplit == 1, "dec_attention: final output needs nsplit == 1");
  static DecAttnKernel prefill4[3] = {{"dec_cross_prefill_kernel<4,4>", dec_cross_prefill_kernel<4, 4>},
                                      {"dec_cross_prefill_kernel<6,4>", dec_cross_prefill_kernel<6, 4>},
                                      {"dec_cross_prefill_kernel<12,4>", dec_cross_prefill_kernel<12, 4>}};
  static DecAttnKernel prefill1[3] = {{"dec_cross_stream_kernel<true,4,true>", dec_cross_stream_kernel<true, 4, true>},
                                      {"dec_cross_stream_kernel<true,6,true>", dec_cross_stream_kernel<true, 6, true>},
                                      {"dec_cross_stream_kernel<true,12,true>", dec_cross_stream_kernel<true, 12, true>}};
  static DecAttnKernel streaming[3] = {{"dec_cross_stream_kernel<true,4,false>", dec_cross_stream_kernel<true, 4>},
                                       {"dec_cross_stream_kernel<true,6,false>", dec_cross_stream_kernel<true, 6>},
                                       {"dec_cross_stream_kernel<true,12,false>", dec_cross_stream_kernel<true, 12>}};
  static DecAttnKernel prefill4_map[3] = {{"dec_cross_prefill_kernel<4,4,true>", dec_cross_prefill_kernel<4, 4, true>},
                                          {"dec_cross_prefill_kernel<6,4,true>", dec_cross_prefill_kernel<6, 4, true>},
                                          {"dec_cross_prefill_kernel<12,4,true>", dec_cross_prefill_kernel<12, 4, true>}};
  static DecAttnKernel prefill1_map[3] = {{"dec_cross_stream_kernel<true,4,true,true>", dec_cross_stream_kernel<true, 4, true, true>},
                                          {"dec_cross_stream_kernel<true,6,true,true>", dec_cross_stream_kernel<true, 6, true, true>},
                                          {"dec_cross_stream_kernel<true,12,true,true>", dec_cross_stream_kernel<true, 12, true, true>}};
  static DecAttnKernel streaming_map[3] = {{"dec_cross_stream_kernel<true,4,false,true>", dec_cross_stream_kernel<true, 4, false, true>},
                                           {"dec_cross_stream_kernel<true,6,false,true>", dec_cross_stream_kernel<true, 6, false, true>},
                                           {"dec_cross_stream_kernel<true,12,false,true>", dec_cross_stream_kernel<true, 12, false, true>}};
  static DecAttnKernel split_kv[2][2] = {
      {{"dec_attention_kernel<false> (cross)", dec_attention_kernel<false>}, {"dec_attention_kernel<true> (cross)", dec_attention_kernel<true>}},
      {{"dec_attention_kernel<false> (self)", dec_attention_kernel<false>}, {"dec_attention_kernel<true> (self)", dec_attention_kernel<true>}}};
  const int np_need = p.pos ? 0 : ((ccx_cdiv(ccx_cdiv(p.T, nsplit), 4) + 31) / 32);
  const int npi = np_need <= 4 ? 0 : (np_need <= 6 ? 1 : 2);
  const bool prefill = p.rows_per_seq > 1 && !p.pos;
  const int pad = p.lds_pad > 0 ? (p.lds_pad < 128 * 1024 ? p.lds_pad : 128 * 1024) : 0;

  DecAttnKernel* k;
  dim3 grid(B * p.H, nsplit);
  int lds = 0;
  if (prefill) {
    CCX_REQUIRE(ctx, nsplit == 1 && final_out && np_need <= 12, "dec_attention: the prefill cross attention takes the whole key range (T <= 1536)");
    CCX_REQUIRE(ctx, !p.kv_map || p.row_seq, "dec_attention: kv_map needs row_seq");
    if (p.kv_map) k = p.rows_per_seq >= 3 ? &prefill4_map[npi] : &prefill1_map[npi];
    else k = p.rows_per_seq >= 3 ? &prefill4[npi] : &prefill1[npi];
    grid = dim3(B * p.H * (p.rows_per_seq >= 3 ? ccx_cdiv(p.rows_per_seq, 4) : p.rows_per_seq), 1);
  } else if (p.stream_mode && !p.pos && np_need <= 12) {
    CCX_REQUIRE(ctx, final_out, "dec_attention: the streaming cross attention takes the whole key range (nsplit 1)");
    k = (p.kv_map && p.row_seq) ? &streaming_map[npi] : &streaming[npi];
    lds = pad;
    CCX_HIP(ctx, k->optin.ensure(ctx->device, (const void*)k->fn, 128 * 1024));
  } else if (p.ind) {
    static DecAttnKernel self_ind = {"dec_attention_kernel<true,true> (self, indirect)", dec_attention_kernel<true, true>};
    CCX_REQUIRE(ctx, p.pos && final_out && !p.row_seq && p.ind_ld >= 1, "dec_attention: the cache indirection is taken by the self attention of a decode step only");
    k = &self_ind;
  } else {
    k = &split_kv[p.pos != nullptr][final_out];
    if (!final_out) lds = pad;
    if (lds > 0) CCX_HIP(ctx, k->optin.ensure(ctx->device, (const void*)k->fn, 128 * 1024));
  }
  {
    const double keys = p.pos ? 1.0 : (double)p.T;
    ccx_prof_scope ps(ctx, stream, k->label, 4.0 * B * p.H * keys * 64 * (prefill ? p.rows_per_seq : 1), (double)B * p.H * keys * 64 * 2 * 2);
    hipLaunchKernelGGL(k->fn, grid, dim3(256), lds, stream, p);
  }
  CCX_CHECK_LAUNCH(ctx);
  return CCX_OK;
}

__device__ __forceinline__ float block_reduce_max(float v, float* sh) {
  v = wave_reduce_max(v);
  const int w = threadIdx.x >> 6, nw = blockDim.x >> 6;
  __syncthreads();
  if ((threadIdx.x & 63) == 0) sh[w] = v;
  __syncthreads();
  float r = sh[0];
  for (int i = 1; i < nw; i++) r = fmaxf(r, sh[i]);
  return r;
}
__device__ __forceinline__ float block_reduce_sum(float v, float* sh) {
  v = wave_reduce_sum(v);
  const int w = threadIdx.x >> 6, nw = blockDim.x >> 6;
  __syncthreads();
  if ((threadIdx.x & 63) == 0) sh[w] = v;
  __syncthreads();
  float r = 0.f;
  for (int i = 0; i < nw; i++) r += sh[i];
  return r;
}

__device__ __forceinline__ uint4 philox4x32_10(uint4 ctr, uint2 key) {
#pragma unroll
  for (int r = 0; r < 10; r++) {
    const unsigned long long p0 = (unsigned long long)0xD2511F53u * ctr.x, p1 = (unsigned long long)0xCD9E8D57u * ctr.z;
    ctr = make_uint4((unsigned)(p1 >> 32) ^ ctr.y ^ key.x, (unsigned)p1, (unsigned)(p0 >> 32) ^ ctr.w ^ key.y, (unsigned)p0);
    key.x += 0x9E3779B9u; key.y += 0xBB67AE85u;
  }
  return ctr;
}
__device__ __forceinline__ float gumbel_from_u32(unsigned x) {
  const float u = ((float)(x >> 8) + 0.5f) * (1.0f / 16777216.0f);
  return -logf(-logf(u));
}

// ... 259 lines not shown
```

### clearconverse_amd/csrc/whisper.hip

```cpp
#include <algorithm>
#include <atomic>
#include <map>
#include <chrono>
#include <math.h>
#include <tuple>
#include "../../include/ccx.h"
#include "align.h"
#include "attention.h"
#include "ccx_common.h"
#include "cross_x.h"
#include "decoder.h"
#include "elementwise.h"
#include "gemm_bf16.h"
#include "logmel.h"
#include "model_store.h"

namespace {

struct EncLayer {
  float *ln1_g, *ln1_b, *ln2_g, *ln2_b;
  bf16_t *Wqkv, *Wo, *W1, *W2;
  float *bqkv, *bo, *b1, *b2;
};
struct DecLayer {
  float *ln1_g, *ln1_b, *lnc_g, *lnc_b, *ln2_g, *ln2_b;
  bf16_t *Wqkv, *Wo, *Wcq, *Wckv, *Wco, *W1, *W2;
  bf16_t* WckT = nullptr;
  bf16_t* Wcq_plain = nullptr;
  bf16_t* Wcq_g = nullptr;
  float *scq = nullptr, *ccq = nullptr;
  float bo_mean = 0.f;
  float *bqkv, *bo, *bcq, *bckv, *bco, *b1, *b2;
  bf16_t *crossK, *crossV, *selfK, *selfV;
};

struct StepPlan {
  int b0, B;
  int sample_len, max_prompt;
  int select;
  int sampling;
  int cross_stream;
  int cross_lds_pad;
  int xs_active;
  int lnfree, xs_fuse_q, fuse_cross_q, xs_full_lines, packed_act;
  int map_on, sid_on;
  int beam_size, beam_maxc;
  int lane_idx;
  int stamp_level;
  int prefill_rows;
  int opt_mask;
  int no_ts;
  int sup_blank;
  int max_init_ts;
  int hist_ngram;
  int hist_pen_bits;
  int bias_on;
  int trunc_on;
  auto tie() const {
    return std::tie(b0, B, sample_len, max_prompt, select, sampling, cross_stream, cross_lds_pad, xs_active, lnfree, xs_fuse_q, fuse_cross_q,
                    xs_full_lines, packed_act, map_on, sid_on, beam_size, beam_maxc, lane_idx, stamp_level, prefill_rows, opt_mask, no_ts, sup_blank,
                    max_init_ts, hist_ngram, hist_pen_bits, bias_on, trunc_on);
  }
  bool operator<(const StepPlan& o) const { return tie() < o.tie(); }
};
static_assert(sizeof(StepPlan) == 29 * sizeof(int) && std::tuple_size<decltype(StepPlan{}.tie())>::value == 29,
              "StepPlan: ints only, and every one of them in tie()");

}

struct ccx_whisper {
  ccx_ctx* ctx = nullptr;
  ccx_whisper_dims d{};
  int max_batch = 0;
  bool finalized = false;
  ccx_whisper* scratch_donor = nullptr;
  int scratch_takers = 0;
  bool destroy_pending = false;
  std::atomic<ccx_whisper*> scratch_owner{nullptr};
  hipEvent_t scratch_free = nullptr;
  ccx_dev_store store{"whisper"};

  int Spad = 0;
  int Vpad = 0;
  int V4 = 0;
  int Fraw = 3008;
  static constexpr int kCrossSplitMax = 8;

  LogmelTables lm{};
  bf16_t *Wc1 = nullptr, *Wc2 = nullptr;
  float *bc1 = nullptr, *bc2 = nullptr, *enc_pos = nullptr, *lnp_g = nullptr, *lnp_b = nullptr;
  std::vector<EncLayer> enc;
  float *tok_emb_f32 = nullptr, *dec_pos = nullptr, *lnd_g = nullptr, *lnd_b = nullptr;
  bf16_t* tok_emb_rm = nullptr;
  std::vector<DecLayer> dec;
  ccx_decode_rules rules{};
  unsigned char* suppress_mask = nullptr;
  bool rules_set = false;
  std::vector<int> rules_suppress;
  ccx_decode_options opts{0, 1, -2, 0, nullptr};
  bool opts_on = false;
  unsigned char* opt_mask = nullptr;
  std::vector<unsigned char> opt_mask_host;
  ccx_decode_history_options hist{1.0f, 0};
  bool bias_on = false;
  int* bias_tab = nullptr;
  ccx_decode_sampling_options trunc{0, 1.0f, 0.0f};

  float* lm_raw = nullptr; unsigned int* lm_max = nullptr; int *lm_n = nullptr, *lm_seek = nullptr, *lm_seg = nullptr;
  bf16_t *im2col = nullptr, *h1 = nullptr, *xn = nullptr, *qb = nullptr, *kb = nullptr, *vtb = nullptr, *attn = nullptr,
         *ffn = nullptr, *xa = nullptr;
  float* x = nullptr;
  float *dx = nullptr, *dx2 = nullptr, *pend = nullptr, *dq = nullptr, *dlogits = nullptr, *part_o = nullptr, *part_ml = nullptr;
  bf16_t *dattn = nullptr, *dffn = nullptr, *dxn = nullptr;
  int *cur_tok = nullptr, *pos = nullptr, *prompt = nullptr, *gen = nullptr, *n_done = nullptr;
  unsigned* sample_cfg = nullptr;
  DecSeqState* state = nullptr;
  int max_prompt_cap = 0, sample_cap = 0;
  static constexpr int kPrefillMax = 16;
// ... 393 lines not shown
    CCX_TRY(w->store.upload(&L.ln2_g, l2g->data.data(), D)); CCX_TRY(w->store.upload(&L.ln2_b, l2b->data.data(), D));
  }

  {
    CCX_NEED(w->store, te, "decoder.token_embedding.weight", d.n_vocab, D);
    CCX_NEED(w->store, pe, "decoder.positional_embedding", d.n_text_ctx, D);
    CCX_NEED(w->store, lg, "decoder.ln.weight", D);
    CCX_NEED(w->store, lb, "decoder.ln.bias", D);
    CCX_TRY(w->store.upload(&w->tok_emb_f32, te->data));
    CCX_TRY(w->store.upload_bf16(&w->tok_emb_rm, te->data.data(), (size_t)d.n_vocab * D));
    CCX_TRY(w->store.upload(&w->dec_pos, pe->data));
    CCX_TRY(w->store.upload(&w->lnd_g, lg->data.data(), D));
    CCX_TRY(w->store.upload(&w->lnd_b, lb->data.data(), D));
  }
  w->dec.resize(d.n_text_layer);
  const int Tc = d.n_text_ctx;
  {
    const char* e = getenv("CCX_CROSS_X");
    w->xs_on = (!e || atoi(e) != 0) && d.n_text_state == D && d.n_text_head == H && ccx_xs_supported(D, H);
    w->kv_cap = w->xs_on ? (B < ccx_whisper::kKvSeqs ? B : ccx_whisper::kKvSeqs) : B;
  }
  for (int l = 0; l < d.n_text_layer; l++) {
    const std::string p = "decoder.blocks." + std::to_string(l) + ".";
    DecLayer& L = w->dec[l];
    CCX_NEED(w->store, qw, p + "attn.query.weight", D, D); CCX_NEED(w->store, qbias, p + "attn.query.bias", D);
    CCX_NEED(w->store, kw, p + "attn.key.weight", D, D);
    CCX_NEED(w->store, vw, p + "attn.value.weight", D, D); CCX_NEED(w->store, vbias, p + "attn.value.bias", D);
    CCX_NEED(w->store, ow, p + "attn.out.weight", D, D); CCX_NEED(w->store, obias, p + "attn.out.bias", D);
    CCX_NEED(w->store, l1g, p + "attn_ln.weight", D); CCX_NEED(w->store, l1b, p + "attn_ln.bias", D);
    CCX_NEED(w->store, cqw, p + "cross_attn.query.weight", D, D); CCX_NEED(w->store, cqb, p + "cross_attn.query.bias", D);
    CCX_NEED(w->store, ckw, p + "cross_attn.key.weight", D, D);
    CCX_NEED(w->store, cvw, p + "cross_attn.value.weight", D, D); CCX_NEED(w->store, cvb, p + "cross_attn.value.bias", D);
    CCX_NEED(w->store, cow, p + "cross_attn.out.weight", D, D); CCX_NEED(w->store, cob, p + "cross_attn.out.bias", D);
    CCX_NEED(w->store, lcg, p + "cross_attn_ln.weight", D); CCX_NEED(w->store, lcb, p + "cross_attn_ln.bias", D);
    CCX_NEED(w->store, m0w, p + "mlp.0.weight", F, D); CCX_NEED(w->store, m0b, p + "mlp.0.bias", F);
    CCX_NEED(w->store, m2w, p + "mlp.2.weight", D, F); CCX_NEED(w->store, m2b, p + "mlp.2.bias", D);
    CCX_NEED(w->store, l2g, p + "mlp_ln.weight", D); CCX_NEED(w->store, l2b, p + "mlp_ln.bias", D);
    std::vector<float> wqkv = cat_rows({&qw->data, &kw->data, &vw->data});
    std::vector<float> bqkv = cat_rows({&qbias->data, &zerosD, &vbias->data});
    std::vector<float> wckv = cat_rows({&ckw->data, &cvw->data});
    std::vector<float> bckv = cat_rows({&zerosD, &cvb->data});
    CCX_TRY(up_bf16_packed(w, &L.Wqkv, wqkv.data(), 3 * D, D, 16)); CCX_TRY(w->store.upload(&L.bqkv, bqkv));
    CCX_TRY(up_bf16_packed(w, &L.Wo, ow->data.data(), D, D, 16)); CCX_TRY(w->store.upload(&L.bo, obias->data.data(), D));
    { double sb = 0.0; for (int k = 0; k < D; k++) sb += obias->data[k]; L.bo_mean = (float)(sb / D); }
    CCX_TRY(up_bf16_packed(w, &L.Wcq, cqw->data.data(), D, D, 16)); CCX_TRY(w->store.upload(&L.bcq, cqb->data.data(), D));
    CCX_TRY(w->store.upload_bf16(&L.Wckv, wckv)); CCX_TRY(w->store.upload(&L.bckv, bckv));
    CCX_TRY(up_bf16_packed(w, &L.Wco, cow->data.data(), D, D, 16)); CCX_TRY(w->store.upload(&L.bco, cob->data.data(), D));
    CCX_TRY(up_bf16_packed(w, &L.W1, m0w->data.data(), F, D, 16)); CCX_TRY(w->store.upload(&L.b1, m0b->data.data(), F));
    CCX_TRY(up_bf16_packed(w, &L.W2, m2w->data.data(), D, F, 16)); CCX_TRY(w->store.upload(&L.b2, m2b->data.data(), D));
    CCX_TRY(w->store.upload(&L.ln1_g, l1g->data.data(), D)); CCX_TRY(w->store.upload(&L.ln1_b, l1b->data.data(), D));
    CCX_TRY(w->store.upload(&L.lnc_g, lcg->data.data(), D)); CCX_TRY(w->store.upload(&L.lnc_b, lcb->data.data(), D));
    CCX_TRY(w->store.upload(&L.ln2_g, l2g->data.data(), D)); CCX_TRY(w->store.upload(&L.ln2_b, l2b->data.data(), D));
    if (w->xs_on) {
      std::vector<float> wkt((size_t)D * D);
      for (int hh = 0; hh < H; hh++)
        for (int f = 0; f < D; f++)
          for (int dd = 0; dd < 64; dd++) wkt[((size_t)hh * D + f) * 64 + dd] = ckw->data[(size_t)(hh * 64 + dd) * D + f];
      CCX_TRY(w->store.upload_bf16(&L.WckT, wkt));
      CCX_TRY(w->store.upload_bf16(&L.Wcq_plain, cqw->data));
      std::vector<float> Wg((size_t)D * D), sv(D), cv(D);
      for (int n = 0; n < D; n++) {
        double ss = 0.0, cc = 0.0;
        for (int k = 0; k < D; k++) {
          const float v = lcg->data[k] * cqw->data[(size_t)n * D + k];
          Wg[(size_t)n * D + k] = v;
          const uint32_t bits = (uint32_t)ccx_host_f32_to_bf16(v) << 16;
          float r;
          memcpy(&r, &bits, 4);
          ss += (double)r;
          cc += (double)lcb->data[k] * (double)cqw->data[(size_t)n * D + k];
        }
        sv[n] = (float)ss;
        cv[n] = (float)(cc + (double)cqb->data[n]);
      }
      CCX_TRY(w->store.upload_bf16(&L.Wcq_g, Wg)); CCX_TRY(w->store.upload(&L.scq, sv)); CCX_TRY(w->store.upload(&L.ccq, cv));
    }
    const size_t ck = (size_t)w->kv_cap * H * w->Spad * 64, sk = (size_t)B * H * Tc * 64;
    CCX_TRY(w->store.alloc(&L.crossK, ck, true)); CCX_TRY(w->store.alloc(&L.crossV, ck, true));
    CCX_TRY(w->store.alloc(&L.selfK, sk, true)); CCX_TRY(w->store.alloc(&L.selfV, sk, true));
  }
  w->store.staged.clear();

  if (ccx_whisper* dn = w->scratch_donor) {
    w->lm_raw = dn->lm_raw; w->lm_max = dn->lm_max; w->lm_n = dn->lm_n; w->lm_seek = dn->lm_seek; w->lm_seg = dn->lm_seg;
    w->im2col = dn->im2col; w->h1 = dn->h1; w->x = dn->x; w->xn = dn->xn;
    w->qb = dn->qb; w->kb = dn->kb; w->vtb = dn->vtb; w->attn = dn->attn; w->ffn = dn->ffn;
  } else {
    CCX_TRY(w->store.alloc(&w->lm_raw, (size_t)B * d.n_mels * w->Fraw, true));
    CCX_TRY(w->store.alloc(&w->lm_max, (size_t)B, true));
    CCX_TRY(w->store.alloc(&w->lm_n, (size_t)B, true));
    CCX_TRY(w->store.alloc(&w->lm_seek, (size_t)B, true));
    CCX_TRY(w->store.alloc(&w->lm_seg, (size_t)B, true));
    CCX_TRY(w->store.alloc(&w->im2col, (size_t)B * 3000 * ccx_logmel_kpad(d.n_mels), true));
    CCX_TRY(w->store.alloc(&w->h1, ((size_t)B * 3002 + 2) * D, true));
    CCX_TRY(w->store.alloc(&w->x, (size_t)B * S * D, true));
    CCX_TRY(w->store.alloc(&w->xn, (size_t)B * S * D, true));
    CCX_TRY(w->store.alloc(&w->qb, (size_t)B * H * w->Spad * 64, true));
    CCX_TRY(w->store.alloc(&w->kb, (size_t)B * H * w->Spad * 64, true));
    CCX_TRY(w->store.alloc(&w->vtb, (size_t)B * H * 64 * w->Spad, true));
    CCX_TRY(w->store.alloc(&w->attn, (size_t)B * S * D, true));
    CCX_TRY(w->store.alloc(&w->ffn, (size_t)B * S * F, true));
  }

  CCX_TRY(w->store.alloc(&w->xa, ((size_t)B * S + 16) * D, true));
  if (w->xs_on) {
    CCX_TRY(w->store.alloc(&w->xq, (size_t)B * H * D, true));
    CCX_TRY(w->store.alloc(&w->pf_xq, (size_t)B * ccx_whisper::kPrefillMax * H * D, true));
    CCX_TRY(w->store.alloc(&w->xs_po, ccx_xs_part_o_elems(B, H, D), true));
    CCX_TRY(w->store.alloc(&w->xs_pml, ccx_xs_part_ml_elems(B), true));
    CCX_TRY(w->store.alloc(&w->pf_xs_po, ccx_xs_part_o_elems((size_t)B * ccx_whisper::kPrefillMax, H, D), true));
    CCX_TRY(w->store.alloc(&w->pf_xs_pml, ccx_xs_part_ml_elems((size_t)B * ccx_whisper::kPrefillMax), true));
    CCX_TRY(w->store.alloc(&w->dxb, (size_t)B * D, true));
    CCX_TRY(w->store.alloc(&w->pf_xb, (size_t)B * ccx_whisper::kPrefillMax * D, true));
    CCX_TRY(w->store.alloc(&w->dst2, (size_t)B * (D / 16), true));
    CCX_TRY(w->store.alloc(&w->pf_st2, (size_t)B * ccx_whisper::kPrefillMax * (D / 16), true));
    CCX_TRY(w->store.alloc(&w->dshift, (size_t)B, true));
    CCX_TRY(w->store.alloc(&w->pf_shift, (size_t)B * ccx_whisper::kPrefillMax, true));
  }
  CCX_TRY(w->store.alloc(&w->dx, (size_t)B * D, true));
  CCX_TRY(w->store.alloc(&w->dx2, (size_t)B * D, true));
  CCX_TRY(w->store.alloc(&w->pend, (size_t)4 * B * D, true));
  CCX_TRY(w->store.alloc(&w->dxn, (size_t)B * D, true));
  CCX_TRY(w->store.alloc(&w->dq, (size_t)B * D, true));
  CCX_TRY(w->store.alloc(&w->dattn, (size_t)B * D, true));
  CCX_TRY(w->store.alloc(&w->dffn, (size_t)B * F, true));
  CCX_TRY(w->store.alloc(&w->dlogits, (size_t)B * w->Vpad, true));
  CCX_TRY(w->store.alloc(&w->part_o, (size_t)B * H * ccx_whisper::kCrossSplitMax * 64, true));
  CCX_TRY(w->store.alloc(&w->part_ml, (size_t)B * H * ccx_whisper::kCrossSplitMax * 2, true));
// ... 75 lines not shown
    CCX_REQUIRE(w->ctx, n_samples[b] >= 0 && n_samples[b] <= stride, "whisper_logmel: n_samples[%d]=%d exceeds stride", b, n_samples[b]);
    const int s = seek ? seek[b] : 0;
    const long need_frames = ((long)n_samples[b] + 200 + 159) / 160 + 1;
    CCX_REQUIRE(w->ctx, need_frames <= w->Fraw, "whisper_logmel: clip %d (%d samples) exceeds the configured maximum of %d frames (ccx_whisper_set_max_audio)", b, n_samples[b], w->Fraw);
    if (need_frames > fcomp) fcomp = need_frames;
    CCX_REQUIRE(w->ctx, s >= 0, "whisper_logmel: negative seek");
    CCX_REQUIRE(w->ctx, !max_frames || max_frames[b] >= 0, "ccx_whisper_logmel_ex: max_frames[%d] = %d is negative", b, max_frames ? max_frames[b] : 0);
  }
  std::vector<int> seg(B), sk(B);
  for (int b = 0; b < B; b++) {
    sk[b] = seek ? seek[b] : 0;
    int sl = n_samples[b] / 160 - sk[b];
    seg[b] = sl < 0 ? 0 : (sl > 3000 ? 3000 : sl);
    if (max_frames && max_frames[b] < seg[b]) seg[b] = max_frames[b];
  }
  CCX_HIP(w->ctx, hipMemcpyAsync(w->lm_n, n_samples, B * 4, hipMemcpyHostToDevice, stream));
  CCX_HIP(w->ctx, hipMemcpyAsync(w->lm_seek, sk.data(), B * 4, hipMemcpyHostToDevice, stream));
  CCX_HIP(w->ctx, hipMemcpyAsync(w->lm_seg, seg.data(), B * 4, hipMemcpyHostToDevice, stream));
  CCX_HIP(w->ctx, hipStreamSynchronize(stream));
  fcomp = (fcomp + 31) / 32 * 32;
  return ccx_launch_logmel(w->ctx, w->lm, audio, stride, w->lm_n, w->lm_seek, w->lm_seg, B, w->Fraw, (int)fcomp, w->lm_raw,
                           w->lm_max, mel_out, w->im2col, stream);
}

int ccx_whisper_set_mel(ccx_whisper* w, const float* mel, int B, void* stream_) {
  if (!w) return CCX_ERR_ARG;
  CCX_REQUIRE(w->ctx, w->finalized && mel && B >= 1 && B <= w->max_batch, "whisper_set_mel: bad arguments");
  CCX_TRY(scratch_acquire(w, (hipStream_t)stream_));
  return ccx_launch_mel_to_im2col(w->ctx, w->d.n_mels, mel, B, w->im2col, (hipStream_t)stream_);
}

static int project_cross_kv(ccx_whisper* w, int n, hipStream_t stream) {
  const ccx_whisper_dims& d = w->d;
  const int D = d.n_audio_state, S = d.n_audio_ctx, H = d.n_audio_head;
  CCX_REQUIRE(w->ctx, n <= w->kv_cap, "whisper: cross K/V caches hold %d sequences, %d asked for", w->kv_cap, n);
  GemmParams p;
  for (int l = 0; l < d.n_text_layer; l++) {
    const DecLayer& L = w->dec[l];
    memset(&p, 0, sizeof(p));
    p.A = w->xa; p.lda = D; p.W = L.Wckv; p.ldw = D; p.M = n * S; p.N = 2 * D; p.K = D; p.bias = L.bckv;
    p.hk = L.crossK; p.hv = L.crossV; p.d_model = D; p.n_head = H; p.S = S; p.Spad = w->Spad; p.v_transposed = 0;
    p.first_block = 1;
    CCX_TRY(ccx_launch_gemm(w->ctx, EPI_HEADS, p, stream));
  }
  w->kv_ready = n;
  return CCX_OK;
}
static void read_chain_switches(StepPlan& p) {
  { const char* e = getenv("CCX_FUSE_CROSS_Q"); p.fuse_cross_q = e ? (atoi(e) != 0) : 1; }
  { const char* e = getenv("CCX_DEC_LNFREE"); p.lnfree = !(e && strcmp(e, "0") == 0); }
  { const char* e = getenv("CCX_XS_FUSE_Q"); p.xs_fuse_q = !e || atoi(e) != 0; }
  p.xs_full_lines = ccx_xs_full_lines_switch();
  p.packed_act = ccx_dec_packed_act_switch();
}
static int select_cross_path(ccx_whisper* w, StepPlan& p, hipStream_t stream, int n_kv = -1) {
  const int B = p.B;
  const char* e = getenv("CCX_CROSS_X_MIN_ROWS");
  const int min_rows = e ? atoi(e) : ccx_whisper::kKvSeqs + 1;
  if (n_kv < 0) n_kv = B;
  p.xs_active = w->xs_on && (B >= min_rows || n_kv > w->kv_cap);
  if (w->xs_on && !p.xs_active && w->kv_ready < n_kv) CCX_TRY(project_cross_kv(w, n_kv, stream));
  return CCX_OK;
}
static StepPlan single_lane_plan(const ccx_whisper* w, int B, int max_prompt) {
  StepPlan p{};
  p.B = B; p.sample_len = 1; p.max_prompt = max_prompt; p.cross_stream = 1;
  p.stamp_level = w->stamps_on ? w->stamp_level : 0;
  read_chain_switches(p);
  return p;
}

int ccx_whisper_encode(ccx_whisper* w, int B, float* xa_out, void* stream_) {
  if (!w) return CCX_ERR_ARG;
  hipStream_t stream = (hipStream_t)stream_;
  ccx_ctx* ctx = w->ctx;
  CCX_REQUIRE(ctx, w->finalized, "whisper: not finalized");
  CCX_REQUIRE(ctx, B >= 1 && B <= w->max_batch, "whisper_encode: B=%d out of range (max %d)", B, w->max_batch);
  const ccx_whisper_dims& d = w->d;
  const int D = d.n_audio_state, F = 4 * D, S = d.n_audio_ctx, H = d.n_audio_head;
  GemmParams p;
  const int KP = ccx_logmel_kpad(d.n_mels);
  memset(&p, 0, sizeof(p));
  p.A = w->im2col; p.lda = KP; p.W = w->Wc1; p.ldw = KP; p.M = B * 3000; p.N = D; p.K = KP;
  p.bias = w->bc1; p.out = w->h1; p.ldo = D; p.rpb_in = 3000; p.rpb_out = 3002; p.roff = 1; p.rpb_valid = 3000;
  CCX_TRY(ccx_launch_gemm(ctx, EPI_BF16_GELU, p, stream));
  memset(&p, 0, sizeof(p));
  p.A = w->h1; p.lda = 2 * D; p.W = w->Wc2; p.ldw = 3 * D; p.M = B * 1501; p.N = D; p.K = 3 * D;
  p.bias = w->bc2; p.out = w->x; p.ldo = D; p.resid = w->enc_pos; p.ldr = D; p.resid_mod = S;
  p.rpb_in = 1501; p.rpb_out = S; p.roff = 0; p.rpb_valid = S;
  CCX_TRY(ccx_launch_gemm(ctx, EPI_F32_GELU_POS, p, stream));

  const int M = B * S;
  for (int l = 0; l < d.n_audio_layer; l++) {
    const EncLayer& L = w->enc[l];
    CCX_TRY(ccx_launch_layernorm(ctx, w->x, D, L.ln1_g, L.ln1_b, w->xn, nullptr, D, M, D, 1e-5f, stream));
    memset(&p, 0, sizeof(p));
    p.A = w->xn; p.lda = D; p.W = L.Wqkv; p.ldw = D; p.M = M; p.N = 3 * D; p.K = D; p.bias = L.bqkv;
    p.hq = w->qb; p.hk = w->kb; p.hv = w->vtb; p.d_model = D; p.n_head = H; p.S = S; p.Spad = w->Spad; p.v_transposed = 1;
    CCX_TRY(ccx_launch_gemm(ctx, EPI_HEADS, p, stream));
    CCX_TRY(ccx_launch_enc_attention(ctx, w->qb, w->kb, w->vtb, w->attn, B, H, S, w->Spad, stream));
    memset(&p, 0, sizeof(p));
    p.A = w->attn; p.lda = D; p.W = L.Wo; p.ldw = D; p.M = M; p.N = D; p.K = D; p.bias = L.bo;
    p.out = w->x; p.ldo = D; p.resid = w->x; p.ldr = D;
    CCX_TRY(ccx_launch_gemm(ctx, EPI_F32_RESID, p, stream));
    CCX_TRY(ccx_launch_layernorm(ctx, w->x, D, L.ln2_g, L.ln2_b, w->xn, nullptr, D, M, D, 1e-5f, stream));
    memset(&p, 0, sizeof(p));
// ... 132 lines not shown
    fill_select_params(w, p, io, bp.sel);
    bp.sel.state = w->state; bp.sel.cur_tok = w->cur_tok; bp.sel.gen = w->gen; bp.sel.x = w->dx;
    bp.beam = p.beam_size; bp.max_cand = p.beam_maxc; bp.cand_id = w->beam_cand_id; bp.cand_lp = w->beam_cand_lp;
    bp.ind = w->beam_ind; bp.ind_ld = d.n_text_ctx; bp.row0 = 0;
    bp.fin_tok = w->beam_fin_tok; bp.fin_score = w->beam_fin_score; bp.fin_n = w->beam_fin_n; bp.fin_count = w->beam_fin_count;
    if (const BeamTrace* t = io.trace) {
      bp.tr_cand_id = t->cid; bp.tr_cand_lp = t->clp; bp.tr_tok = t->tok; bp.tr_parent = t->par; bp.tr_score = t->score; bp.tr_rows = B;
    }
    CCX_TRY(ccx_launch_dec_beam(ctx, bp, B / p.beam_size, io.stream));
  } else if (p.select) {
    DecSelectParams sp;
    memset(&sp, 0, sizeof(sp));
    fill_select_params(w, p, io, sp);
    sp.state = w->state + b0; sp.prompt = w->prompt + ro * p.max_prompt; sp.max_prompt = p.max_prompt;
    sp.cur_tok = w->cur_tok + b0; sp.gen = w->gen + ro * p.sample_len; sp.x = w->dx + ro * D;
    sp.sample_cfg = w->sample_cfg; sp.row0 = b0; sp.sample = p.sampling ? 1 : 0;
    sp.trunc = p.trunc_on;
    sp.stream_id = p.sid_on ? w->row_sid + b0 : nullptr;
    CCX_TRY(ccx_launch_dec_select(ctx, sp, B, io.stream));
  }
  return CCX_OK;
}

int dec_step(ccx_whisper* w, const StepPlan& p, const StepIo& io) {
  ccx_ctx* ctx = w->ctx;
  const ccx_whisper_dims& d = w->d;
  const int D = d.n_text_state, F = 4 * D, H = d.n_text_head, Tc = d.n_text_ctx;
  const float scale_log2e = 0.125f * 1.4426950408889634f;
  const int b0 = p.b0, nseq = p.B, prefill_rows = p.prefill_rows, lane_idx = p.lane_idx;
  const bool pre = prefill_rows > 0, map_on = p.map_on != 0, xs_active = p.xs_active != 0;
  const int B = pre ? nseq * prefill_rows : nseq;
  const int ns = cross_split(nseq, H, p.cross_stream != 0);
  const long pstride = (long)B * D;
  const long ro = b0;
  hipStream_t stream = io.stream;
  float* cur = pre ? w->pf_x : w->dx + ro * D;
  float* other = pre ? w->pf_x2 : w->dx2 + ro * D;
  float* pend = pre ? w->pf_pend : w->pend + 4 * ro * D;
  float* dq = pre ? w->pf_q : w->dq + ro * D;
  bf16_t* dxn = pre ? w->pf_xn : w->dxn + ro * D;
  bf16_t* dattn = pre ? w->pf_attn : w->dattn + ro * D;
  bf16_t* dffn = pre ? w->pf_ffn : w->dffn + ro * F;
  float* part_o = w->part_o + ro * H * ccx_whisper::kCrossSplitMax * 64;
  float* part_ml = w->part_ml + ro * H * ccx_whisper::kCrossSplitMax * 2;
  int* pos = pre ? w->pf_pos : w->pos + b0;
  const int* row_seq = pre ? w->pf_seq : nullptr;
  const int* win = !map_on ? nullptr : (pre ? w->pf_win : w->row_win + b0);
  const long cross_off = map_on ? 0 : ro * H * w->Spad * 64, self_off = ro * H * Tc * 64;
  auto stamp = [&](int tag, int level) {
    if (level <= p.stamp_level)
      hipLaunchKernelGGL(dec_stamp_kernel, dim3(1), dim3(1), 0, stream, w->stamps + (size_t)lane_idx * ccx_whisper::kStampCap,
                         w->stamp_count + lane_idx, ccx_whisper::kStampCap, tag);
  };
  const int packed = (p.packed_act && B > 16 && B % 16 == 0) ? 1 : 0;
  int pend_n = 0;
  auto ln_linear = [&](int epi, const bf16_t* W, const float* bias, int N, const float* g, const float* bta, void* out, long ldo,
                       DecLinearParams* extra) -> int {
    DecLinearParams lp;
    if (extra) lp = *extra; else memset(&lp, 0, sizeof(lp));
    lp.M = B; lp.N = N; lp.K = D; lp.W = W; lp.ldw = D; lp.bias = bias; lp.out = out; lp.ldo = ldo;
    int rc;
    if (B > 16) {
      rc = ccx_launch_dec_resolve_ln(ctx, cur, pend, pend_n, pstride, g, bta, dxn, pend_n > 0 ? other : nullptr, B, D, 1e-5f, stream,
                                     lp.ln_mean_out, packed);
      if (rc) return rc;
      lp.ln_mean_out = nullptr;
      lp.act = dxn; lp.lda = D; lp.act_packed = packed;
      rc = ccx_launch_dec_linear(ctx, ACT_BF16, epi, lp, stream);
    } else {
      lp.x = cur; lp.pend = pend; lp.pend_n = pend_n; lp.pend_stride = pstride; lp.x_out = pend_n > 0 ? other : nullptr;
      lp.ln_g = g; lp.ln_b = bta; lp.eps = 1e-5f;
      rc = ccx_launch_dec_linear(ctx, ACT_LN, epi, lp, stream);
    }
    if (rc) return rc;
    if (pend_n > 0) { float* t = cur; cur = other; other = t; pend_n = 0; }
    return CCX_OK;
  };
  auto partial_linear = [&](int act, const bf16_t* W, const float* bias, int K, const bf16_t* a, int a_packed = 0) -> int {
    DecLinearParams lp;
    memset(&lp, 0, sizeof(lp));
    lp.M = B; lp.N = D; lp.K = K; lp.W = W; lp.ldw = K; lp.bias = bias; lp.act = a; lp.lda = K; lp.act_packed = a_packed;
    lp.part_o = part_o; lp.part_ml = part_ml; lp.nsplit = ns;
    lp.out = pend; lp.ldo = D; lp.pend_stride = pstride;
    int rc = ccx_launch_dec_linear(ctx, act, DEPI_PARTIAL, lp, stream);
    if (rc) return rc;
    pend_n = ccx_dec_linear_ksplit(K, DEPI_PARTIAL);
    return CCX_OK;
  };
  const bool lnfree = xs_active && p.lnfree;
  const bool xs_fused = xs_active && !lnfree && p.xs_fuse_q;
  const bool fuse_q = !xs_active && p.fuse_cross_q && !pre && B <= 16 && D == 768 && !map_on;
  const bool q_launch = !fuse_q && !lnfree && !xs_fused;
  bf16_t* xb = !lnfree ? nullptr : (pre ? w->pf_xb : w->dxb + ro * D);
  float2* st2 = !lnfree ? nullptr : (pre ? w->pf_st2 : w->dst2 + ro * (D / 16));
  float* shift = !lnfree ? nullptr : (pre ? w->pf_shift : w->dshift + ro);
  for (int l = 0; l < d.n_text_layer; l++) {
    const DecLayer& L = w->dec[l];
    {
      DecLinearParams ex;
      memset(&ex, 0, sizeof(ex));
      ex.cache_k = L.selfK + self_off; ex.cache_v = L.selfV + self_off; ex.cache_T = Tc; ex.pos = pos; ex.row_seq = row_seq;
      ex.ln_mean_out = shift;
      CCX_TRY(ln_linear(DEPI_SELF_QKV, L.Wqkv, L.bqkv, 3 * D, L.ln1_g, L.ln1_b, dq, D, &ex));
      stamp(16, 2);
    }
    DecAttnParams ap;
    memset(&ap, 0, sizeof(ap));
    ap.q = dq; ap.k = L.selfK + self_off; ap.v = L.selfV + self_off; ap.H = H; ap.kv_T = Tc; ap.pos = pos; ap.scale_log2e = scale_log2e;
    ap.out_bf16 = dattn; ap.row_seq = row_seq;
    if (p.beam_size > 0 && !pre) { ap.ind = w->beam_ind; ap.ind_ld = Tc; }
    CCX_TRY(ccx_launch_dec_attention(ctx, ap, B, 1, true, stream));
    stamp(17, 2);
    if (lnfree) {
      DecLinearParams lp;
      memset(&lp, 0, sizeof(lp));
      lp.M = B; lp.N = D; lp.K = D; lp.W = L.Wo; lp.ldw = D; lp.bias = L.bo; lp.act = dattn; lp.lda = D;
      lp.xres = cur; lp.xb = xb; lp.st_out = st2; lp.shift = shift; lp.shift_c = L.bo_mean;
      CCX_TRY(ccx_launch_dec_linear(ctx, ACT_BF16, DEPI_RESOLVE, lp, stream));
    } else {
      CCX_TRY(partial_linear(ACT_BF16, L.Wo, L.bo, D, dattn));
    }
    stamp(18, 2);
    if (q_launch) CCX_TRY(ln_linear(DEPI_F32, L.Wcq, L.bcq, D, L.lnc_g, L.lnc_b, dq, D, nullptr));
    if (io.align) CCX_TRY(align_scores_hook(w, *io.align, l, dq, B, stream));
    stamp(1, 1);
    if (l == 0 && io.stagger) CCX_HIP(ctx, hipEventRecord(io.stagger, stream));
    if (xs_active) {
      XsParams xp;
      memset(&xp, 0, sizeof(xp));
      if (lnfree) {
        xp.xb = xb; xp.ln_stats = st2; xp.ln_s = L.scq; xp.Wq = L.Wcq_g; xp.bq = L.ccq; xp.eps = 1e-5f;
      } else if (xs_fused) {
        xp.x = cur; xp.pend = pend; xp.pend_n = pend_n; xp.pend_stride = pstride; xp.x_out = pend_n > 0 ? other : nullptr;
        xp.ln_g = L.lnc_g; xp.ln_b = L.lnc_b; xp.eps = 1e-5f; xp.Wq = L.Wcq_plain; xp.bq = L.bcq;
      }
      xp.q = dq; xp.WkT = L.WckT; xp.xq = pre ? w->pf_xq : w->xq + ro * H * D;
      xp.part_o = pre ? w->pf_xs_po : w->xs_po + ccx_xs_part_o_elems(ro, H, D);
      xp.part_ml = pre ? w->pf_xs_pml : w->xs_pml + ccx_xs_part_ml_elems(ro);
      xp.X = (pre || map_on) ? w->xa : w->xa + ro * (long)d.n_audio_ctx * D; xp.x_seq_stride = (long)d.n_audio_ctx * D;
      xp.row_seq = map_on ? win : row_seq;
      xp.Wv = L.Wckv + (long)D * D; xp.bv = L.bckv + D; xp.out = dattn;
      xp.rows = B; xp.H = H; xp.S = d.n_audio_ctx; xp.D = D; xp.scale_log2e = scale_log2e;
      xp.lds_pad = (p.cross_lds_pad > 0 && !pre) ? 65536 : 0;
      xp.rows_per_seq = pre ? prefill_rows : 0;
      xp.full_lines = p.xs_full_lines;
      CCX_TRY(ccx_launch_xs_cross_attention(ctx, xp, stream));
      if (xs_fused && pend_n > 0) { float* t = cur; cur = other; other = t; pend_n = 0; }
      stamp(2, 1);
      CCX_TRY(partial_linear(ACT_BF16, L.Wco, L.bco, D, dattn));
      stamp(19, 2);
    } else {
      memset(&ap, 0, sizeof(ap));
      ap.q = dq; ap.k = L.crossK + cross_off; ap.v = L.crossV + cross_off; ap.H = H; ap.kv_T = w->Spad; ap.pos = nullptr; ap.T = d.n_audio_ctx;
      ap.scale_log2e = scale_log2e; ap.part_o = part_o; ap.part_ml = part_ml; ap.out_bf16 = dattn;
      ap.lds_pad = p.cross_lds_pad;
      ap.stream_mode = (p.cross_stream && B > 16) ? 1 : 0;
      ap.row_seq = win; ap.kv_map = map_on ? 1 : 0;
      if (fuse_q) {
        ap.qx = cur; ap.q_pend = pend; ap.q_pend_n = pend_n; ap.q_pend_stride = pstride; ap.q_x_out = pend_n > 0 ? other : nullptr;
        ap.q_ln_g = L.lnc_g; ap.q_ln_b = L.lnc_b; ap.q_eps = 1e-5f; ap.q_W = L.Wcq; ap.q_bias = L.bcq; ap.q_K = D;
        CCX_TRY(ccx_launch_dec_cross_fused_q(ctx, ap, B, ns, stream));
        if (pend_n > 0) { float* t = cur; cur = other; other = t; pend_n = 0; }
        CCX_TRY(partial_linear(ACT_COMBINE, L.Wco, L.bco, D, nullptr));
      } else if (pre) {
        if (!map_on) ap.row_seq = prefill_rows > 1 ? row_seq : nullptr;
        ap.rows_per_seq = prefill_rows > 1 ? prefill_rows : 0;
        ap.lds_pad = 0; ap.stream_mode = 1;
        CCX_TRY(ccx_launch_dec_attention(ctx, ap, nseq, 1, true, stream));
        CCX_TRY(partial_linear(ACT_BF16, L.Wco, L.bco, D, dattn));
      } else if (B > 16) {
        CCX_TRY(ccx_launch_dec_attention(ctx, ap, B, ns, ns == 1, stream));
        stamp(2, 1);
        if (ns > 1) CCX_TRY(ccx_launch_dec_combine(ctx, part_o, part_ml, ns, dattn, B, H, stream));
        CCX_TRY(partial_linear(ACT_BF16, L.Wco, L.bco, D, dattn));
        stamp(19, 2);
      } else {
        CCX_TRY(ccx_launch_dec_attention(ctx, ap, B, ns, false, stream));
        CCX_TRY(partial_linear(ACT_COMBINE, L.Wco, L.bco, D, nullptr));
      }
    }
    {
      DecLinearParams ex;
      memset(&ex, 0, sizeof(ex));
      ex.out_packed = packed;
      CCX_TRY(ln_linear(DEPI_BF16_GELU, L.W1, L.b1, F, L.ln2_g, L.ln2_b, dffn, F, &ex));
    }
    stamp(20, 2);
    CCX_TRY(partial_linear(ACT_BF16, L.W2, L.b2, F, dffn, packed));
    stamp(21, 2);
  }
  CCX_TRY(ccx_launch_dec_resolve_ln(ctx, cur, pend, pend_n, pstride, w->lnd_g, w->lnd_b, dxn, nullptr, B, D, 1e-5f, stream));
  if (pre) return CCX_OK;
  CCX_TRY(dec_head(w, p, io));
  stamp(3, 1);
  return CCX_OK;
}

int upload_decode_state(ccx_whisper* w, const int32_t* prompt_ids, const int32_t* prompt_lens, int max_prompt, int B,
                        float temperature, uint64_t seed, hipStream_t stream, bool prefilled = false) {
  std::vector<DecSeqState> st(B);
  std::vector<int> tok(B), ps(B, 0);
  for (int b = 0; b < B; b++) {
// ... 788 lines not shown
```

### include/ccx.h

```cpp
#ifndef CCX_H
#define CCX_H
#include <stdint.h>
#ifdef __cplusplus
extern "C" {
#endif

#define CCX_DTYPE_F32 0
#define CCX_DTYPE_BF16 1
#define CCX_DTYPE_F16 2

typedef struct ccx_ctx ccx_ctx;
typedef struct ccx_whisper ccx_whisper;

const char* ccx_version(void);
int ccx_ctx_create(int device, ccx_ctx** out);
void ccx_ctx_destroy(ccx_ctx* ctx);
const char* ccx_last_error(const ccx_ctx* ctx);

int ccx_prof_enable(ccx_ctx* ctx, int on);
int ccx_prof_count(ccx_ctx* ctx);
int ccx_prof_get(ccx_ctx* ctx, int i, char* name_out, int name_cap, double* flops, double* bytes, float* ms);


int ccx_gemm_bf16(ccx_ctx* ctx, int epi, const void* A_dev, int64_t lda, const void* W_dev, int64_t ldw,
// ... 161 lines not shown
  int rows_per_seq;
  int nsplit, combine;
  int lds_pad;
  const void* x; const void* pend; int pend_n; int64_t pend_stride;
  const void* ln_g; const void* ln_b; float eps;
  const float* wq_host; const void* bq;
  void* out; void* part_o; void* part_ml; void* q_x_out;
  int64_t q_elems, kv_elems, out_elems, part_o_elems, part_ml_elems, x_elems, pend_elems, q_x_out_elems;
  const uint16_t* ind; int ind_ld;
} ccx_dec_attn_desc;

int ccx_dec_attention_desc(ccx_ctx* ctx, int form, const ccx_dec_attn_desc* desc, void* stream);

typedef struct ccx_dec_seq_state {
  int pos, prompt_len, n_gen, done;
  int last_tok, pen_tok, last_ts_tok, n_tokens;
  float sum_logprob, no_speech_prob;
} ccx_dec_seq_state;

typedef struct ccx_dec_select_desc {
  const void* logits; int64_t ld; int n_vocab; int B;
  const ccx_decode_rules* rules;
  ccx_dec_seq_state* state;
  const int* prompt; int max_prompt;
  int sample_len;
  int* gen;
  int* cur_tok; int* pos;
  int* n_done;
  const void* tok_emb; const void* pos_emb; void* x; int D;
  int sample; float temperature; uint64_t seed; int row0;
  int64_t logits_elems, tok_emb_elems, pos_emb_elems, x_elems;
  const int* stream_ids;
  const ccx_decode_options* opts;
  const ccx_decode_sampling_options* sampling;
  float* cut_out; int* kept_out; float* kept_mass_out;
} ccx_dec_select_desc;

int ccx_dec_select_step(ccx_ctx* ctx, const ccx_dec_select_desc* desc, void* stream);

#define CCX_DEC_EPI_PARTIAL 0
#define CCX_DEC_EPI_F32 1
#define CCX_DEC_EPI_SELF_QKV 2
#define CCX_DEC_EPI_GELU 3
typedef struct ccx_dec_ln_linear_desc {
  int M, K, F, N, epi, packed;
  const void* x; const void* ln_g; const void* ln_b; float eps;
  const float* w1_host; const void* b1;
  const float* w_host; const void* bias;
  void* out;
  int64_t x_elems, out_elems;
} ccx_dec_ln_linear_desc;
int ccx_dec_ln_linear(ccx_ctx* ctx, const ccx_dec_ln_linear_desc* desc, void* stream);

typedef struct ccx_dec_beam_desc {
  const void* logits; int64_t ld; int n_vocab;
  int G, beam_size, max_candidates;
  const ccx_decode_rules* rules;
  ccx_dec_seq_state* state;
  int sample_len;
  int* hist; int* cur_tok; int* pos; int* n_done;
  const void* tok_emb; const void* pos_emb; void* x; int D;
  uint16_t* ind; int ind_ld;
  int* fin_tok; float* fin_score; int* fin_n; int* fin_count;
  int* cand_id; float* cand_lp; int* tok_out; int* parent_out;
  int64_t logits_elems, tok_emb_elems, pos_emb_elems, x_elems;
  const ccx_decode_options* opts;
} ccx_dec_beam_desc;
int ccx_dec_beam_step(ccx_ctx* ctx, const ccx_dec_beam_desc* desc, void* stream);

typedef struct ccx_dec_history_desc {
  void* logits; int64_t logits_elems;
  int64_t ld; int n_vocab; int rows;
  const ccx_dec_seq_state* state;
  const int* hist; int sample_len;
  int text_end;
  float repetition_penalty; int no_repeat_ngram_size;
} ccx_dec_history_desc;
int ccx_dec_history_step(ccx_ctx* ctx, const ccx_dec_history_desc* desc, void* stream);

typedef struct ccx_dec_bias_desc {
  void* logits; int64_t logits_elems;
  int64_t ld; int n_vocab; int rows;
  const ccx_dec_seq_state* state;
  const int* hist; int sample_len;
  int text_end;
  ccx_decode_bias_options table;
} ccx_dec_bias_desc;
int ccx_dec_bias_step(ccx_ctx* ctx, const ccx_dec_bias_desc* desc, void* stream);

typedef struct ccx_dec_token_probs_desc {
  const void* logits; int64_t logits_elems;
  int64_t ld; int n_vocab; int rows;
  int lo, hi, pick;
  int* argmax; float* pick_prob;
  void* probs; int64_t probs_elems;
} ccx_dec_token_probs_desc;
int ccx_dec_token_probs(ccx_ctx* ctx, const ccx_dec_token_probs_desc* desc, void* stream);

typedef struct ccx_dec_pick_probs_desc {
  const void* logits; int64_t logits_elems;
  int64_t ld; int rows; int hi;
  const void* picks; int64_t picks_elems; int64_t pick_stride;
  void* out; int64_t out_elems; int64_t out_stride;
} ccx_dec_pick_probs_desc;
int ccx_dec_pick_probs(ccx_ctx* ctx, const ccx_dec_pick_probs_desc* desc, void* stream);

// ... 207 lines not shown
```

Before: 1830.

## Pack decoder mid-chain activations and cross-attention weights into MFMA fragment layout

Stores the cross-attention key, value and folded query weights in MFMA fragment order, so each lane reads contiguous 16-byte chunks instead of strided rows. It also lets the self-attention output, Wo resolve, X-stream cross attention and cross-output linear pass activations in a packed fragment image when the batch is a multiple of 16 in a plain greedy decode. The goal is more coalesced global loads in the decoder step's middle chain. It adds a test entry point plus shared host helpers, and the packed path depends on several consistency conditions across kernels.

```diff
diff --git a/clearconverse_amd/_lib.py b/clearconverse_amd/_lib.py
--- a/clearconverse_amd/_lib.py
+++ b/clearconverse_amd/_lib.py
@@ -69,6 +69,19 @@
 DEC_ATTN_SELF, DEC_ATTN_SPLIT, DEC_ATTN_STREAM, DEC_ATTN_PREFILL, DEC_ATTN_FUSED_Q, DEC_ATTN_TWO_LAUNCH_Q = range(6)
 DEC_ATTN_STREAM_MAPPED = 7
 DEC_ATTN_SELF_IND = 8
+
+
+class DecMidChainDesc(C.Structure):
+    _fields_ = [
+        ("M", C.c_int), ("D", C.c_int), ("H", C.c_int), ("S", C.c_int), ("kv_T", C.c_int), ("packed", C.c_int),
+        ("q", C.c_void_p), ("self_k", C.c_void_p), ("self_v", C.c_void_p), ("x", C.c_void_p), ("shift", C.c_void_p), ("xa", C.c_void_p),
+        ("pos", C.c_void_p),
+        ("wo", C.c_void_p), ("bo", C.c_void_p),
+        ("lnc_g", C.c_void_p), ("lnc_b", C.c_void_p), ("cq_w", C.c_void_p), ("cq_b", C.c_void_p),
+        ("ck_w", C.c_void_p), ("cv_w", C.c_void_p), ("cv_b", C.c_void_p),
+        ("co_w", C.c_void_p), ("co_b", C.c_void_p),
+        ("out", C.c_void_p), ("packed_used", C.POINTER(C.c_int)),
+        ("q_elems", C.c_int64), ("kv_elems", C.c_int64), ("x_elems", C.c_int64), ("xa_elems", C.c_int64), ("out_elems", C.c_int64)]
 
 
 class DecLnLinearDesc(C.Structure):
@@ -316,6 +329,8 @@
     "ccx_whisper_decode_greedy": (_i, [_vp, _i32p, _i32p, _i, _i, _i, _i32p, _i32p, _fp, _fp, _vp]),
     "ccx_dec_attention_desc": (_i, [_vp, _i, C.POINTER(DecAttnDesc), _vp]),
     "ccx_dec_ln_linear": (_i, [_vp, C.POINTER(DecLnLinearDesc), _vp]),
+    "ccx_dec_mid_chain_out_elems": (_i64, [_i, _i, _i]),
+    "ccx_dec_mid_chain": (_i, [_vp, C.POINTER(DecMidChainDesc), _vp]),
     "ccx_dec_select_step": (_i, [_vp, C.POINTER(DecSelectDesc), _vp]),
     "ccx_dec_beam_step": (_i, [_vp, C.POINTER(DecBeamDesc), _vp]),
     "ccx_whisper_decode_beam": (_i, [_vp, _i32p, _i32p, _i, _i, _i32p, _i, _i, _i, _i, _i32p, _i32p, _fp, _i32p, _fp,
diff --git a/clearconverse_amd/csrc/cross_x.h b/clearconverse_amd/csrc/cross_x.h
--- a/clearconverse_amd/csrc/cross_x.h
+++ b/clearconverse_amd/csrc/cross_x.h
@@ -1,4 +1,6 @@
 #pragma once
+#include <cstring>
+#include <vector>
 #include "ccx_common.h"
 
 struct XsParams {
@@ -24,9 +26,37 @@
   float scale_log2e;
   int lds_pad;
   int full_lines;
+  int xb_packed, out_packed;
 };
 
+
 int ccx_xs_full_lines_switch();
+
+static inline void ccx_xs_fold_query_ln(const float* gamma, const float* beta, const float* wq, const float* bq, int D, std::vector<float>& Wg,
+                                        std::vector<float>& s, std::vector<float>& c) {
+  Wg.resize((size_t)D * D); s.resize(D); c.resize(D);
+  for (int n = 0; n < D; n++) {
+    double ss = 0.0, cc = 0.0;
+    for (int k = 0; k < D; k++) {
+      const float v = gamma[k] * wq[(size_t)n * D + k];
+      Wg[(size_t)n * D + k] = v;
+      const uint32_t bits = (uint32_t)ccx_host_f32_to_bf16(v) << 16;
+      float r;
+      memcpy(&r, &bits, 4);
+      ss += (double)r;
+      cc += (double)beta[k] * (double)wq[(size_t)n * D + k];
+    }
+    s[n] = (float)ss;
+    c[n] = (float)(cc + (double)bq[n]);
+  }
+}
+static inline std::vector<float> ccx_xs_relay_key(const float* wk, int H, int D) {
+  std::vector<float> wkt((size_t)H * D * 64);
+  for (int hh = 0; hh < H; hh++)
+    for (int f = 0; f < D; f++)
+      for (int dd = 0; dd < 64; dd++) wkt[((size_t)hh * D + f) * 64 + dd] = wk[(size_t)(hh * 64 + dd) * D + f];
+  return wkt;
+}
 
 #define XS_SPLIT 2
 static inline size_t ccx_xs_part_o_elems(size_t rows, int H, int D) { return rows * XS_SPLIT * (size_t)H * D; }
diff --git a/clearconverse_amd/csrc/cross_x.hip b/clearconverse_amd/csrc/cross_x.hip
--- a/clearconverse_amd/csrc/cross_x.hip
+++ b/clearconverse_amd/csrc/cross_x.hip
@@ -1,5 +1,6 @@
 #include "cross_x.h"
 #include "dec_ln.h"
+#include "decoder.h"
 
 namespace {
 
@@ -27,12 +28,12 @@
     const float4* src = (const float4*)(p.q + (long)row * D + h * 64 + ks * 32 + g * 8);
     qb[ks] = pack8(src[0], src[1]);
   }
-  const bf16_t* wbase = p.WkT + ((long)h * D + wave * FW + n) * 64 + g * 8;
+  const bf16_t* wbase = p.WkT + ((long)h * D + wave * FW) * 64 + lane * 8;
   bf16_t* dst = p.xq + ((long)row * p.H + h) * D + wave * FW + g * 4;
 #pragma unroll
   for (int mt = 0; mt < NMT; mt++) {
     const bf16x8 a0 = *(const bf16x8*)(wbase + (long)mt * 16 * 64);
-    const bf16x8 a1 = *(const bf16x8*)(wbase + (long)mt * 16 * 64 + 32);
+    const bf16x8 a1 = *(const bf16x8*)(wbase + (long)mt * 16 * 64 + 512);
     f32x4 c = {0.f, 0.f, 0.f, 0.f};
     c = __builtin_amdgcn_mfma_f32_16x16x32_bf16(a0, qb[0], c, 0, 0, 0);
     c = __builtin_amdgcn_mfma_f32_16x16x32_bf16(a1, qb[1], c, 0, 0, 0);
@@ -51,9 +52,9 @@
   const int wave = threadIdx.x >> 6, lane = threadIdx.x & 63, n = lane & 15, g = lane >> 4;
   bf16x8 wq[NKS];
   {
-    const bf16_t* wsrc = p.Wq + (long)(h * 64 + wave * 16 + n) * D + g * 8;
-#pragma unroll
-    for (int ks = 0; ks < NKS; ks++) wq[ks] = *(const bf16x8*)(wsrc + ks * 32);
+    const bf16_t* wsrc = p.Wq + ((long)(h * 4 + wave) * NKS * 64 + lane) * 8;
+#pragma unroll
+    for (int ks = 0; ks < NKS; ks++) wq[ks] = *(const bf16x8*)(wsrc + ks * 512);
   }
   {
     float4 gg[NI], bb[NI];
@@ -111,12 +112,12 @@
       else ca = __builtin_amdgcn_mfma_f32_16x16x32_bf16(wq[ks], b, ca, 0, 0, 0);
     }
   }
-  const bf16_t* wbase = p.WkT + ((long)h * D + wave * FW + n) * 64 + g * 8;
+  const bf16_t* wbase = p.WkT + ((long)h * D + wave * FW) * 64 + lane * 8;
   bf16x8 wk[NMT][2];
 #pragma unroll
   for (int mt = 0; mt < NMT; mt++) {
     wk[mt][0] = *(const bf16x8*)(wbase + (long)mt * 16 * 64);
-    wk[mt][1] = *(const bf16x8*)(wbase + (long)mt * 16 * 64 + 32);
+    wk[mt][1] = *(const bf16x8*)(wbase + (long)mt * 16 * 64 + 512);
   }
   {
     const float4 bias = *(const float4*)(p.bq + h * 64 + wave * 16 + g * 4);
@@ -148,12 +149,13 @@
   if (!live) row = p.rows - 1;
   bf16x8 wq[NKS], xb[NKS];
   {
-    const bf16_t* wsrc = p.Wq + (long)(h * 64 + wave * 16 + n) * D + g * 8;
-    const bf16_t* xsrc = p.xb + (long)row * D + g * 8;
-#pragma unroll
-    for (int ks = 0; ks < NKS; ks++) wq[ks] = *(const bf16x8*)(wsrc + ks * 32);
-#pragma unroll
-    for (int ks = 0; ks < NKS; ks++) xb[ks] = *(const bf16x8*)(xsrc + ks * 32);
+    const bf16_t* wsrc = p.Wq + ((long)(h * 4 + wave) * NKS * 64 + lane) * 8;
+    const bf16_t* xsrc = p.xb_packed ? p.xb + ((long)blockIdx.y * NKS * 64 + lane) * 8 : p.xb + (long)row * D + g * 8;
+    const int xstep = p.xb_packed ? 512 : 32;
+#pragma unroll
+    for (int ks = 0; ks < NKS; ks++) wq[ks] = *(const bf16x8*)(wsrc + ks * 512);
+#pragma unroll
+    for (int ks = 0; ks < NKS; ks++) xb[ks] = *(const bf16x8*)(xsrc + ks * xstep);
   }
   if (threadIdx.x < 64) {
     const int r = threadIdx.x >> 2, qt = threadIdx.x & 3;
@@ -173,12 +175,12 @@
     const float var = fmaf(-mean, mean, s2 / (float)D);
     if (qt == 0) st_s[r] = make_float2(mean, rsqrtf(fmaxf(var, 0.f) + p.eps));
   }
-  const bf16_t* wbase = p.WkT + ((long)h * D + wave * FW + n) * 64 + g * 8;
+  const bf16_t* wbase = p.WkT + ((long)h * D + wave * FW) * 64 + lane * 8;
   bf16x8 wk[NMT][2];
 #pragma unroll
   for (int mt = 0; mt < NMT; mt++) {
     wk[mt][0] = *(const bf16x8*)(wbase + (long)mt * 16 * 64);
-    wk[mt][1] = *(const bf16x8*)(wbase + (long)mt * 16 * 64 + 32);
+    wk[mt][1] = *(const bf16x8*)(wbase + (long)mt * 16 * 64 + 512);
   }
   const float4 cc = *(const float4*)(p.bq + h * 64 + wave * 16 + g * 4);
   const float4 ss = *(const float4*)(p.ln_s + h * 64 + wave * 16 + g * 4);
@@ -214,12 +216,12 @@
   const int h = blockIdx.x, r0 = blockIdx.y * 16;
   const int wave = threadIdx.x >> 6, lane = threadIdx.x & 63, n = lane & 15, g = lane >> 4;
   const int o0 = h * 64 + wave * 16;
-  const bf16_t* wsrc = p.Wv + (long)(o0 + n) * D + g * 8;
+  const bf16_t* wsrc = p.Wv + ((long)(h * 4 + wave) * NKS * 64 + lane) * 8;
   constexpr int CH = NKS % 6 == 0 ? 6 : 4;
   static_assert(NKS % CH == 0, "D must be a multiple of 128");
   bf16x8 a[CH];
 #pragma unroll
-  for (int k = 0; k < CH; k++) a[k] = *(const bf16x8*)(wsrc + k * 32);
+  for (int k = 0; k < CH; k++) a[k] = *(const bf16x8*)(wsrc + k * 512);
   {
     const int rr = threadIdx.x >> 4, c = threadIdx.x & 15;
     int row = r0 + rr;
@@ -263,7 +265,7 @@
     bf16x8 an[CH];
     if (c0 + CH < NKS) {
 #pragma unroll
-      for (int k = 0; k < CH; k++) an[k] = *(const bf16x8*)(wsrc + (c0 + CH + k) * 32);
+      for (int k = 0; k < CH; k++) an[k] = *(const bf16x8*)(wsrc + (c0 + CH + k) * 512);
     }
 #pragma unroll
     for (int k = 0; k < CH; k++) {
@@ -280,7 +282,8 @@
   if (row < p.rows) {
     const float4 bias = *(const float4*)(p.bv + o0 + g * 4);
     const float v0 = ca[0] + cb[0] + bias.x, v1 = ca[1] + cb[1] + bias.y, v2 = ca[2] + cb[2] + bias.z, v3 = ca[3] + cb[3] + bias.w;
-    *(u32x2*)(p.out + (long)row * D + o0 + g * 4) = (u32x2){pack_bf16x2(v0, v1), pack_bf16x2(v2, v3)};
+    bf16_t* o = p.out + (p.out_packed ? dec_frag_off(row, o0 + g * 4, D >> 5) : (long)row * D + o0 + g * 4);
+    *(u32x2*)o = (u32x2){pack_bf16x2(v0, v1), pack_bf16x2(v2, v3)};
   }
 }
 
@@ -574,6 +577,8 @@
   CCX_REQUIRE(ctx, !p.xb || (p.ln_stats && p.ln_s && p.Wq && p.bq), "xs cross attention: bad LayerNorm-free query arguments");
   CCX_REQUIRE(ctx, !p.x || (p.pend && p.ln_g && p.ln_b && p.Wq && p.bq && p.pend_n >= 0 && p.pend_n <= 4 && p.x_out != p.x), "xs cross attention: bad fused-query arguments");
   CCX_REQUIRE(ctx, p.part_o && p.part_ml, "xs cross attention: partial buffers missing");
+  CCX_REQUIRE(ctx, !(p.xb_packed || p.out_packed) || p.rows % 16 == 0, "xs cross attention: fragment images need rows=%d to be a multiple of 16", p.rows);
+  CCX_REQUIRE(ctx, !p.xb_packed || p.xb, "xs cross attention: xb_packed without xb");
   switch (p.D) {
     case 128: return launch_xs<128>(ctx, p, stream);
     case 256: return launch_xs<256>(ctx, p, stream);
@@ -606,11 +611,8 @@
     for (int i = 0; i < rows; i++)
       CCX_REQUIRE(ctx, row_seq_host[i] == row_seq_host[i - i % rows_per_seq], "cross_attention_xa: row %d is not in its group's sequence", i);
   }
-  std::vector<bf16_t> wkt((size_t)D * D), wv((size_t)D * D);
-  for (int hh = 0; hh < H; hh++)
-    for (int f = 0; f < D; f++)
-      for (int dd = 0; dd < 64; dd++) wkt[((size_t)hh * D + f) * 64 + dd] = ccx_host_f32_to_bf16(wk_host[(size_t)(hh * 64 + dd) * D + f]);
-  for (size_t i = 0; i < wv.size(); i++) wv[i] = ccx_host_f32_to_bf16(wv_host[i]);
+  const std::vector<float> wkt_f = ccx_xs_relay_key(wk_host, H, D);
+  const std::vector<bf16_t> wkt = pack_mfma_rows(wkt_f.data(), H * D, 64, 16), wv = pack_mfma_rows(wv_host, D, D, 16);
   bf16_t *d_wkt = nullptr, *d_wv = nullptr, *d_xq = nullptr, *d_out = nullptr;
   float *d_bv = nullptr, *d_po = nullptr, *d_pml = nullptr;
   int* d_rs = nullptr;
diff --git a/clearconverse_amd/csrc/dec_ops.hip b/clearconverse_amd/csrc/dec_ops.hip
--- a/clearconverse_amd/csrc/dec_ops.hip
+++ b/clearconverse_amd/csrc/dec_ops.hip
@@ -1,6 +1,7 @@
 #include "../../include/ccx.h"
 #include "ccx_common.h"
 #include "decoder.h"
+#include "cross_x.h"
 #include "op_scratch.h"
 
 static_assert(sizeof(ccx_dec_seq_state) == sizeof(DecSeqState), "ccx_dec_seq_state mirrors DecSeqState field for field");
@@ -255,6 +256,115 @@
       hipLaunchKernelGGL(dec_ops_rows_to_f32_kernel, dim3((unsigned)((n + 255) / 256)), dim3(256), 0, stream, d_g16, (float*)d->out, M, N, packed);
       DO_HIP(hipGetLastError());
     }
+  }
+  DO_HIP(hipStreamSynchronize(stream));
+  return rc;
+}
+
+extern "C" int64_t ccx_dec_mid_chain_out_elems(int M, int D, int H) {
+  return (int64_t)M * D * 5 + (int64_t)M * (D / 16) * 2 + (int64_t)M * H * D;
+}
+
+extern "C" int ccx_dec_mid_chain(ccx_ctx* ctx, const ccx_dec_mid_chain_desc* d, void* stream_) {
+  if (!ctx) return CCX_ERR_ARG;
+  hipStream_t stream = (hipStream_t)stream_;
+  CCX_REQUIRE(ctx, d != nullptr, "ccx_dec_mid_chain: desc is NULL");
+  const int M = d->M, D = d->D, H = d->H, S = d->S, Tc = d->kv_T;
+  CCX_REQUIRE(ctx, M >= 1 && M <= 4096, "ccx_dec_mid_chain: M = %d out of range [1, 4096]", M);
+  CCX_REQUIRE(ctx, H >= 1 && H <= 64 && D == 64 * H && ccx_xs_supported(D, H), "ccx_dec_mid_chain: D = %d with H = %d heads is not a width the X-stream kernels have (D == 64 H, H in {2, 4, 6, 8, 12})", D, H);
+  CCX_REQUIRE(ctx, S >= 16 && S <= 4096, "ccx_dec_mid_chain: S = %d out of range [16, 4096]", S);
+  CCX_REQUIRE(ctx, Tc >= 1 && Tc <= 4096, "ccx_dec_mid_chain: kv_T = %d out of range [1, 4096]", Tc);
+  CCX_REQUIRE(ctx, d->packed == 0 || d->packed == 1, "ccx_dec_mid_chain: packed = %d must be 0 or 1", d->packed);
+  CCX_REQUIRE(ctx, d->q && d->self_k && d->self_v && d->x && d->xa && d->out && d->pos && d->packed_used, "ccx_dec_mid_chain: q, self_k, self_v, x, xa, pos, out or packed_used is NULL");
+  CCX_REQUIRE(ctx, d->wo && d->bo && d->lnc_g && d->lnc_b && d->cq_w && d->cq_b && d->ck_w && d->cv_w && d->cv_b && d->co_w && d->co_b, "ccx_dec_mid_chain: a host weight is NULL");
+  CCX_REQUIRE(ctx, ccx_aligned16(d->q) && ccx_aligned16(d->self_k) && ccx_aligned16(d->self_v) && ccx_aligned16(d->x) && ccx_aligned16(d->shift) && ccx_aligned16(d->xa) && ccx_aligned16(d->out),
+              "ccx_dec_mid_chain: q, self_k, self_v, x, shift, xa or out not 16-byte aligned");
+  for (int i = 0; i < M; i++) CCX_REQUIRE(ctx, d->pos[i] >= 0 && d->pos[i] < Tc, "ccx_dec_mid_chain: pos[%d] = %d out of range [0, kv_T = %d)", i, d->pos[i], Tc);
+  const int64_t MD = (int64_t)M * D;
+  CCX_REQUIRE(ctx, MD <= d->q_elems, "ccx_dec_mid_chain: q is read up to element %ld, q_elems=%ld", (long)MD, (long)d->q_elems);
+  CCX_REQUIRE(ctx, MD * Tc <= d->kv_elems, "ccx_dec_mid_chain: self_k / self_v are read up to element %ld, kv_elems=%ld", (long)(MD * Tc), (long)d->kv_elems);
+  CCX_REQUIRE(ctx, MD <= d->x_elems, "ccx_dec_mid_chain: x is read up to element %ld, x_elems=%ld", (long)MD, (long)d->x_elems);
+  CCX_REQUIRE(ctx, MD * S <= d->xa_elems, "ccx_dec_mid_chain: xa is read up to element %ld, xa_elems=%ld", (long)(MD * S), (long)d->xa_elems);
+  const int64_t n_out = ccx_dec_mid_chain_out_elems(M, D, H);
+  CCX_REQUIRE(ctx, n_out <= d->out_elems, "ccx_dec_mid_chain: out is written up to element %ld, out_elems=%ld", (long)n_out, (long)d->out_elems);
+
+  const int pk = ccx_dec_rows_as_image(d->packed, M);
+  *d->packed_used = pk;
+  float* o_attn = (float*)d->out;
+  float* o_x = o_attn + MD;
+  float* o_xb = o_x + MD;
+  float* o_st = o_xb + MD;
+  float* o_xq = o_st + (int64_t)M * (D / 16) * 2;
+  float* o_cross = o_xq + MD * H;
+  float* o_co = o_cross + MD;
+
+  ccx_op_scratch sc;
+  const size_t Mp = (size_t)(M + 15) / 16 * 16;
+  bf16_t *d_attn = nullptr, *d_xb = nullptr, *d_xq = nullptr, *d_wo = nullptr, *d_wco = nullptr, *d_wg = nullptr, *d_wkt = nullptr, *d_wv = nullptr;
+  float *d_bo = nullptr, *d_bco = nullptr, *d_s = nullptr, *d_c = nullptr, *d_bv = nullptr, *d_po = nullptr, *d_pml = nullptr;
+  float2* d_st = nullptr; int* d_pos = nullptr;
+  DO_HIP(hipMemsetAsync(d->out, 0xFF, (size_t)n_out * 4, stream));
+  DO_HIP(sc.alloc(&d_attn, Mp * D)); DO_HIP(hipMemsetAsync(d_attn, 0xFF, Mp * D * 2, stream));
+  DO_HIP(sc.alloc(&d_xb, Mp * D)); DO_HIP(hipMemsetAsync(d_xb, 0xFF, Mp * D * 2, stream));
+  DO_HIP(sc.alloc(&d_st, (size_t)M * (D / 16))); DO_HIP(hipMemsetAsync(d_st, 0xFF, (size_t)M * (D / 16) * 8, stream));
+  DO_HIP(sc.alloc(&d_xq, (size_t)MD * H)); DO_HIP(hipMemsetAsync(d_xq, 0xFF, (size_t)MD * H * 2, stream));
+  DO_HIP(sc.alloc(&d_po, ccx_xs_part_o_elems(M, H, D))); DO_HIP(hipMemsetAsync(d_po, 0xFF, ccx_xs_part_o_elems(M, H, D) * 4, stream));
+  DO_HIP(sc.alloc(&d_pml, ccx_xs_part_ml_elems(M))); DO_HIP(hipMemsetAsync(d_pml, 0xFF, ccx_xs_part_ml_elems(M) * 4, stream));
+  DO_HIP(sc.upload(&d_pos, d->pos, (size_t)M));
+  float bo_mean;
+  {
+    const std::vector<bf16_t> wo = pack_mfma_rows(d->wo, D, D, 16), wco = pack_mfma_rows(d->co_w, D, D, 16), wv = pack_mfma_rows(d->cv_w, D, D, 16);
+    const std::vector<float> wkt_f = ccx_xs_relay_key(d->ck_w, H, D);
+    const std::vector<bf16_t> wkt = pack_mfma_rows(wkt_f.data(), H * D, 64, 16);
+    std::vector<float> Wg, sv, cv;
+    ccx_xs_fold_query_ln(d->lnc_g, d->lnc_b, d->cq_w, d->cq_b, D, Wg, sv, cv);
+    const std::vector<bf16_t> wg = pack_mfma_rows(Wg.data(), D, D, 16);
+    double sb = 0.0;
+    for (int k = 0; k < D; k++) sb += d->bo[k];
+    bo_mean = (float)(sb / D);
+    DO_HIP(sc.upload(&d_wo, wo.data(), wo.size())); DO_HIP(sc.upload(&d_wco, wco.data(), wco.size())); DO_HIP(sc.upload(&d_wv, wv.data(), wv.size()));
+    DO_HIP(sc.upload(&d_wkt, wkt.data(), wkt.size())); DO_HIP(sc.upload(&d_wg, wg.data(), wg.size()));
+    DO_HIP(sc.upload(&d_s, sv.data(), sv.size())); DO_HIP(sc.upload(&d_c, cv.data(), cv.size()));
+    DO_HIP(sc.upload(&d_bo, d->bo, (size_t)D)); DO_HIP(sc.upload(&d_bco, d->co_b, (size_t)D)); DO_HIP(sc.upload(&d_bv, d->cv_b, (size_t)D));
+  }
+  const float scale_log2e = 0.125f * 1.4426950408889634f;
+  const dim3 cgrid((unsigned)((MD + 255) / 256));
+  DecAttnParams ap;
+  memset(&ap, 0, sizeof(ap));
+  ap.q = (const float*)d->q; ap.k = (const bf16_t*)d->self_k; ap.v = (const bf16_t*)d->self_v; ap.H = H; ap.kv_T = Tc; ap.pos = d_pos;
+  ap.scale_log2e = scale_log2e; ap.out_bf16 = d_attn; ap.out_packed = pk;
+  int rc = ccx_launch_dec_attention(ctx, ap, M, 1, true, stream);
+  if (rc == CCX_OK) { hipLaunchKernelGGL(dec_ops_rows_to_f32_kernel, cgrid, dim3(256), 0, stream, d_attn, o_attn, M, D, pk); DO_HIP(hipGetLastError()); }
+  if (rc == CCX_OK) {
+    DO_HIP(hipMemcpyAsync(o_x, d->x, (size_t)MD * 4, hipMemcpyDeviceToDevice, stream));
+    DecLinearParams lp;
+    memset(&lp, 0, sizeof(lp));
+    lp.M = M; lp.N = D; lp.K = D; lp.W = d_wo; lp.ldw = D; lp.bias = d_bo; lp.act = d_attn; lp.lda = D; lp.act_packed = pk; lp.out_packed = pk;
+    lp.xres = o_x; lp.xb = d_xb; lp.st_out = d_st; lp.shift = (const float*)d->shift; lp.shift_c = bo_mean;
+    rc = ccx_launch_dec_linear(ctx, ACT_BF16, DEPI_RESOLVE, lp, stream);
+  }
+  if (rc == CCX_OK) {
+    hipLaunchKernelGGL(dec_ops_rows_to_f32_kernel, cgrid, dim3(256), 0, stream, d_xb, o_xb, M, D, pk); DO_HIP(hipGetLastError());
+    DO_HIP(hipMemcpyAsync(o_st, d_st, (size_t)M * (D / 16) * 8, hipMemcpyDeviceToDevice, stream));
+    XsParams xp;
+    memset(&xp, 0, sizeof(xp));
+    xp.xb = d_xb; xp.xb_packed = pk; xp.ln_stats = d_st; xp.ln_s = d_s; xp.Wq = d_wg; xp.bq = d_c; xp.eps = 1e-5f;
+    xp.WkT = d_wkt; xp.xq = d_xq; xp.part_o = d_po; xp.part_ml = d_pml;
+    xp.X = (const bf16_t*)d->xa; xp.x_seq_stride = (long)S * D;
+    xp.Wv = d_wv; xp.bv = d_bv; xp.out = d_attn; xp.out_packed = pk;
+    xp.rows = M; xp.H = H; xp.S = S; xp.D = D; xp.scale_log2e = scale_log2e; xp.full_lines = ccx_xs_full_lines_switch();
+    rc = ccx_launch_xs_cross_attention(ctx, xp, stream);
+  }
+  if (rc == CCX_OK) {
+    const long nq = (long)MD * H;
+    hipLaunchKernelGGL(dec_ops_bf16_to_f32_kernel, dim3((unsigned)((nq + 255) / 256)), dim3(256), 0, stream, d_xq, o_xq, nq);
+    hipLaunchKernelGGL(dec_ops_rows_to_f32_kernel, cgrid, dim3(256), 0, stream, d_attn, o_cross, M, D, pk);
+    DO_HIP(hipGetLastError());
+    DecLinearParams lp;
+    memset(&lp, 0, sizeof(lp));
+    lp.M = M; lp.N = D; lp.K = D; lp.W = d_wco; lp.ldw = D; lp.bias = d_bco; lp.act = d_attn; lp.lda = D; lp.act_packed = pk;
+    lp.out = o_co; lp.ldo = D; lp.pend_stride = (long)MD;
+    rc = ccx_launch_dec_linear(ctx, ACT_BF16, DEPI_PARTIAL, lp, stream);
   }
   DO_HIP(hipStreamSynchronize(stream));
   return rc;
diff --git a/clearconverse_amd/csrc/decoder.h b/clearconverse_amd/csrc/decoder.h
--- a/clearconverse_amd/csrc/decoder.h
+++ b/clearconverse_amd/csrc/decoder.h
@@ -33,6 +33,8 @@
   return (((long)(m >> 4) * ksteps + (k >> 5)) * 64 + (((k >> 3) & 3) * 16 + (m & 15))) * 8 + (k & 7);
 }
 int ccx_dec_packed_act_switch();
+int ccx_dec_packed_mid_switch();
+static inline int ccx_dec_rows_as_image(int on, int rows) { return (on && rows > 16 && rows % 16 == 0) ? 1 : 0; }
 
 struct DecAttnParams {
   const float* q;
@@ -53,6 +55,7 @@
   const bf16_t* q_W; const float* q_bias; int q_K;
   int kv_map;
   const unsigned short* ind; int ind_ld;
+  int out_packed;
 };
 int ccx_launch_dec_attention(ccx_ctx* ctx, const DecAttnParams& p, int B, int nsplit, bool final_out, hipStream_t stream);
 int ccx_launch_dec_cross_fused_q(ccx_ctx* ctx, const DecAttnParams& p, int B, int nsplit, hipStream_t stream);
diff --git a/clearconverse_amd/csrc/decoder.hip b/clearconverse_amd/csrc/decoder.hip
--- a/clearconverse_amd/csrc/decoder.hip
+++ b/clearconverse_amd/csrc/decoder.hip
@@ -276,7 +276,7 @@
         *(float4*)(p.xres + (long)m * p.N + n) = make_float4(v[0], v[1], v[2], v[3]);
         uint2 pk;
         pk.x = pack_bf16x2(c0, c1); pk.y = pack_bf16x2(c2, c3);
-        *(uint2*)(p.xb + (long)m * p.N + n) = pk;
+        *(uint2*)(p.xb + (p.out_packed ? dec_frag_off(m, n, p.N >> 5) : (long)m * p.N + n)) = pk;
         if ((ln >> 4) == 0) p.st_out[(long)m * (p.N >> 4) + (n >> 4)] = make_float2(s1, s2);
       }
       continue;
@@ -467,6 +467,11 @@
   return !(e && strcmp(e, "0") == 0);
 }
 
+int ccx_dec_packed_mid_switch() {
+  const char* e = getenv("CCX_DEC_PACKED_MID");
+  return !(e && strcmp(e, "0") == 0);
+}
+
 int ccx_dec_linear_ksplit(int K, int epi) {
   if (epi == DEPI_RESOLVE) return 1;
   int ks = ccx_cdiv(K, 1024);
@@ -480,7 +485,8 @@
   CCX_REQUIRE(ctx, act == ACT_BF16 || p.K <= 1280, "dec_linear: LN/combine activation needs K <= 1280");
   CCX_REQUIRE(ctx, p.pend_n >= 0 && p.pend_n <= 4, "dec_linear: at most 4 pending slabs");
   CCX_REQUIRE(ctx, !p.act_packed || act == ACT_BF16, "dec_linear: act_packed is taken with bf16 activations only");
-  CCX_REQUIRE(ctx, !p.out_packed || (act == ACT_BF16 && epi == DEPI_BF16_GELU && p.N % 32 == 0), "dec_linear: out_packed needs the GELU epilogue and N=%d a multiple of 32", p.N);
+  CCX_REQUIRE(ctx, !p.out_packed || (act == ACT_BF16 && (epi == DEPI_BF16_GELU || epi == DEPI_RESOLVE) && p.N % 32 == 0),
+              "dec_linear: out_packed needs the GELU or the resolve epilogue and N=%d a multiple of 32", p.N);
   const int ksplit = ccx_dec_linear_ksplit(p.K, epi);
   CCX_REQUIRE(ctx, epi == DEPI_PARTIAL || ksplit == 1, "dec_linear: K=%d needs a split-K (partial) epilogue", p.K);
   CCX_REQUIRE(ctx, ksplit <= 4, "dec_linear: K=%d would leave %d partial slabs (at most 4)", p.K, ksplit);
@@ -614,7 +620,7 @@
   }
 }
 
-template <bool FINAL, bool IND = false>
+template <bool FINAL, bool IND = false, bool IMG = false>
 __global__ __launch_bounds__(256) void dec_attention_kernel(DecAttnParams p) {
   __shared__ float sm_m[4][8], sm_l[4][8], sm_o[4][8][8];
   const int tid = threadIdx.x, lane = tid & 63, wave = tid >> 6;
@@ -678,7 +684,7 @@
     float mx, l, o;
     soft_merge_waves(sm_m, sm_l, sm_o, tid, mx, l, o);
     if (FINAL) {
-      p.out_bf16[((long)b * p.H + h) * 64 + tid] = f32_to_bf16(o / l);
+      p.out_bf16[IMG ? dec_frag_off(b, h * 64 + tid, p.H * 2) : ((long)b * p.H + h) * 64 + tid] = f32_to_bf16(o / l);
     } else {
       const long pbase = ((long)b * p.H + h) * gridDim.y + split;
       p.part_o[pbase * 64 + tid] = o;
@@ -1010,6 +1016,8 @@
   static DecAttnKernel split_kv[2][2] = {
       {{"dec_attention_kernel<false> (cross)", dec_attention_kernel<false>}, {"dec_attention_kernel<true> (cross)", dec_attention_kernel<true>}},
       {{"dec_attention_kernel<false> (self)", dec_attention_kernel<false>}, {"dec_attention_kernel<true> (self)", dec_attention_kernel<true>}}};
+  CCX_REQUIRE(ctx, !p.out_packed || (p.pos && final_out && nsplit == 1 && !p.row_seq && !p.ind && !p.stream_mode && p.rows_per_seq <= 1 && B % 16 == 0),
+              "dec_attention: out_packed is taken by the self attention of a decode step (pos, nsplit 1, no row_seq, no ind) over whole 16-row tiles only (B=%d, nsplit=%d)", B, nsplit);
   const int np_need = p.pos ? 0 : ((ccx_cdiv(ccx_cdiv(p.T, nsplit), 4) + 31) / 32);
   const int npi = np_need <= 4 ? 0 : (np_need <= 6 ? 1 : 2);
   const bool prefill = p.rows_per_seq > 1 && !p.pos;
@@ -1029,6 +1037,9 @@
     k = (p.kv_map && p.row_seq) ? &streaming_map[npi] : &streaming[npi];
     lds = pad;
     CCX_HIP(ctx, k->optin.ensure(ctx->device, (const void*)k->fn, 128 * 1024));
+  } else if (p.out_packed) {
+    static DecAttnKernel self_image = {"dec_attention_kernel<true,false,true> (self, image)", dec_attention_kernel<true, false, true>};
+    k = &self_image;
   } else if (p.ind) {
     static DecAttnKernel self_ind = {"dec_attention_kernel<true,true> (self, indirect)", dec_attention_kernel<true, true>};
     CCX_REQUIRE(ctx, p.pos && final_out && !p.row_seq && p.ind_ld >= 1, "dec_attention: the cache indirection is taken by the self attention of a decode step only");
diff --git a/clearconverse_amd/csrc/whisper.hip b/clearconverse_amd/csrc/whisper.hip
--- a/clearconverse_amd/csrc/whisper.hip
+++ b/clearconverse_amd/csrc/whisper.hip
@@ -27,6 +27,7 @@
   bf16_t *Wqkv, *Wo, *Wcq, *Wckv, *Wco, *W1, *W2;
   bf16_t* WckT = nullptr;
   bf16_t* Wcq_plain = nullptr;
+  bf16_t* Wcv_x = nullptr;
   bf16_t* Wcq_g = nullptr;
   float *scq = nullptr, *ccq = nullptr;
   float bo_mean = 0.f;
@@ -42,7 +43,7 @@
   int cross_stream;
   int cross_lds_pad;
   int xs_active;
-  int lnfree, xs_fuse_q, fuse_cross_q, xs_full_lines, packed_act;
+  int lnfree, xs_fuse_q, fuse_cross_q, xs_full_lines, packed_act, packed_mid;
   int map_on, sid_on;
   int beam_size, beam_maxc;
   int lane_idx;
@@ -58,12 +59,12 @@
   int trunc_on;
   auto tie() const {
     return std::tie(b0, B, sample_len, max_prompt, select, sampling, cross_stream, cross_lds_pad, xs_active, lnfree, xs_fuse_q, fuse_cross_q,
-                    xs_full_lines, packed_act, map_on, sid_on, beam_size, beam_maxc, lane_idx, stamp_level, prefill_rows, opt_mask, no_ts, sup_blank,
+                    xs_full_lines, packed_act, packed_mid, map_on, sid_on, beam_size, beam_maxc, lane_idx, stamp_level, prefill_rows, opt_mask, no_ts, sup_blank,
                     max_init_ts, hist_ngram, hist_pen_bits, bias_on, trunc_on);
   }
   bool operator<(const StepPlan& o) const { return tie() < o.tie(); }
 };
-static_assert(sizeof(StepPlan) == 29 * sizeof(int) && std::tuple_size<decltype(StepPlan{}.tie())>::value == 29,
+static_assert(sizeof(StepPlan) == 30 * sizeof(int) && std::tuple_size<decltype(StepPlan{}.tie())>::value == 30,
               "StepPlan: ints only, and every one of them in tie()");
 
 }
@@ -563,28 +564,13 @@
     CCX_TRY(w->store.upload(&L.lnc_g, lcg->data.data(), D)); CCX_TRY(w->store.upload(&L.lnc_b, lcb->data.data(), D));
     CCX_TRY(w->store.upload(&L.ln2_g, l2g->data.data(), D)); CCX_TRY(w->store.upload(&L.ln2_b, l2b->data.data(), D));
     if (w->xs_on) {
-      std::vector<float> wkt((size_t)D * D);
-      for (int hh = 0; hh < H; hh++)
-        for (int f = 0; f < D; f++)
-          for (int dd = 0; dd < 64; dd++) wkt[((size_t)hh * D + f) * 64 + dd] = ckw->data[(size_t)(hh * 64 + dd) * D + f];
-      CCX_TRY(w->store.upload_bf16(&L.WckT, wkt));
-      CCX_TRY(w->store.upload_bf16(&L.Wcq_plain, cqw->data));
-      std::vector<float> Wg((size_t)D * D), sv(D), cv(D);
-      for (int n = 0; n < D; n++) {
-        double ss = 0.0, cc = 0.0;
-        for (int k = 0; k < D; k++) {
-          const float v = lcg->data[k] * cqw->data[(size_t)n * D + k];
-          Wg[(size_t)n * D + k] = v;
-          const uint32_t bits = (uint32_t)ccx_host_f32_to_bf16(v) << 16;
-          float r;
-          memcpy(&r, &bits, 4);
-          ss += (double)r;
-          cc += (double)lcb->data[k] * (double)cqw->data[(size_t)n * D + k];
-        }
-        sv[n] = (float)ss;
-        cv[n] = (float)(cc + (double)cqb->data[n]);
-      }
-      CCX_TRY(w->store.upload_bf16(&L.Wcq_g, Wg)); CCX_TRY(w->store.upload(&L.scq, sv)); CCX_TRY(w->store.upload(&L.ccq, cv));
+      const std::vector<float> wkt = ccx_xs_relay_key(ckw->data.data(), H, D);
+      CCX_TRY(up_bf16_packed(w, &L.WckT, wkt.data(), H * D, 64, 16));
+      L.Wcq_plain = L.Wcq;
+      CCX_TRY(up_bf16_packed(w, &L.Wcv_x, cvw->data.data(), D, D, 16));
+      std::vector<float> Wg, sv, cv;
+      ccx_xs_fold_query_ln(lcg->data.data(), lcb->data.data(), cqw->data.data(), cqb->data.data(), D, Wg, sv, cv);
+      CCX_TRY(up_bf16_packed(w, &L.Wcq_g, Wg.data(), D, D, 16)); CCX_TRY(w->store.upload(&L.scq, sv)); CCX_TRY(w->store.upload(&L.ccq, cv));
     }
     const size_t ck = (size_t)w->kv_cap * H * w->Spad * 64, sk = (size_t)B * H * Tc * 64;
     CCX_TRY(w->store.alloc(&L.crossK, ck, true)); CCX_TRY(w->store.alloc(&L.crossV, ck, true));
@@ -766,6 +752,7 @@
   { const char* e = getenv("CCX_XS_FUSE_Q"); p.xs_fuse_q = !e || atoi(e) != 0; }
   p.xs_full_lines = ccx_xs_full_lines_switch();
   p.packed_act = ccx_dec_packed_act_switch();
+  p.packed_mid = ccx_dec_packed_mid_switch();
 }
 static int select_cross_path(ccx_whisper* w, StepPlan& p, hipStream_t stream, int n_kv = -1) {
   const int B = p.B;
@@ -1004,7 +991,8 @@
       hipLaunchKernelGGL(dec_stamp_kernel, dim3(1), dim3(1), 0, stream, w->stamps + (size_t)lane_idx * ccx_whisper::kStampCap,
                          w->stamp_count + lane_idx, ccx_whisper::kStampCap, tag);
   };
-  const int packed = (p.packed_act && B > 16 && B % 16 == 0) ? 1 : 0;
+  const int packed = ccx_dec_rows_as_image(p.packed_act, B);
+  const int packed_mid = (ccx_dec_rows_as_image(p.packed_mid, B) && !pre && !map_on && p.beam_size == 0 && xs_active && p.lnfree) ? 1 : 0;
   int pend_n = 0;
   auto ln_linear = [&](int epi, const bf16_t* W, const float* bias, int N, const float* g, const float* bta, void* out, long ldo,
                        DecLinearParams* extra) -> int {
@@ -1061,12 +1049,14 @@
     ap.q = dq; ap.k = L.selfK + self_off; ap.v = L.selfV + self_off; ap.H = H; ap.kv_T = Tc; ap.pos = pos; ap.scale_log2e = scale_log2e;
     ap.out_bf16 = dattn; ap.row_seq = row_seq;
     if (p.beam_size > 0 && !pre) { ap.ind = w->beam_ind; ap.ind_ld = Tc; }
+    ap.out_packed = packed_mid;
     CCX_TRY(ccx_launch_dec_attention(ctx, ap, B, 1, true, stream));
     stamp(17, 2);
     if (lnfree) {
       DecLinearParams lp;
       memset(&lp, 0, sizeof(lp));
       lp.M = B; lp.N = D; lp.K = D; lp.W = L.Wo; lp.ldw = D; lp.bias = L.bo; lp.act = dattn; lp.lda = D;
+      lp.act_packed = packed_mid; lp.out_packed = packed_mid;
       lp.xres = cur; lp.xb = xb; lp.st_out = st2; lp.shift = shift; lp.shift_c = L.bo_mean;
       CCX_TRY(ccx_launch_dec_linear(ctx, ACT_BF16, DEPI_RESOLVE, lp, stream));
     } else {
@@ -1081,7 +1071,7 @@
       XsParams xp;
       memset(&xp, 0, sizeof(xp));
       if (lnfree) {
-        xp.xb = xb; xp.ln_stats = st2; xp.ln_s = L.scq; xp.Wq = L.Wcq_g; xp.bq = L.ccq; xp.eps = 1e-5f;
+        xp.xb = xb; xp.xb_packed = packed_mid; xp.ln_stats = st2; xp.ln_s = L.scq; xp.Wq = L.Wcq_g; xp.bq = L.ccq; xp.eps = 1e-5f;
       } else if (xs_fused) {
         xp.x = cur; xp.pend = pend; xp.pend_n = pend_n; xp.pend_stride = pstride; xp.x_out = pend_n > 0 ? other : nullptr;
         xp.ln_g = L.lnc_g; xp.ln_b = L.lnc_b; xp.eps = 1e-5f; xp.Wq = L.Wcq_plain; xp.bq = L.bcq;
@@ -1091,7 +1081,7 @@
       xp.part_ml = pre ? w->pf_xs_pml : w->xs_pml + ccx_xs_part_ml_elems(ro);
       xp.X = (pre || map_on) ? w->xa : w->xa + ro * (long)d.n_audio_ctx * D; xp.x_seq_stride = (long)d.n_audio_ctx * D;
       xp.row_seq = map_on ? win : row_seq;
-      xp.Wv = L.Wckv + (long)D * D; xp.bv = L.bckv + D; xp.out = dattn;
+      xp.Wv = L.Wcv_x; xp.bv = L.bckv + D; xp.out = dattn; xp.out_packed = packed_mid;
       xp.rows = B; xp.H = H; xp.S = d.n_audio_ctx; xp.D = D; xp.scale_log2e = scale_log2e;
       xp.lds_pad = (p.cross_lds_pad > 0 && !pre) ? 65536 : 0;
       xp.rows_per_seq = pre ? prefill_rows : 0;
@@ -1099,7 +1089,7 @@
       CCX_TRY(ccx_launch_xs_cross_attention(ctx, xp, stream));
       if (xs_fused && pend_n > 0) { float* t = cur; cur = other; other = t; pend_n = 0; }
       stamp(2, 1);
-      CCX_TRY(partial_linear(ACT_BF16, L.Wco, L.bco, D, dattn));
+      CCX_TRY(partial_linear(ACT_BF16, L.Wco, L.bco, D, dattn, packed_mid));
       stamp(19, 2);
     } else {
       memset(&ap, 0, sizeof(ap));
diff --git a/include/ccx.h b/include/ccx.h
--- a/include/ccx.h
+++ b/include/ccx.h
@@ -237,6 +237,21 @@
 } ccx_dec_ln_linear_desc;
 int ccx_dec_ln_linear(ccx_ctx* ctx, const ccx_dec_ln_linear_desc* desc, void* stream);
 
+typedef struct ccx_dec_mid_chain_desc {
+  int M, D, H, S, kv_T, packed;
+  const void* q; const void* self_k; const void* self_v; const void* x; const void* shift; const void* xa;
+  const int* pos;
+  const float* wo; const float* bo;
+  const float* lnc_g; const float* lnc_b; const float* cq_w; const float* cq_b;
+  const float* ck_w; const float* cv_w; const float* cv_b;
+  const float* co_w; const float* co_b;
+  void* out;
+  int* packed_used;
+  int64_t q_elems, kv_elems, x_elems, xa_elems, out_elems;
+} ccx_dec_mid_chain_desc;
+int64_t ccx_dec_mid_chain_out_elems(int M, int D, int H);
+int ccx_dec_mid_chain(ccx_ctx* ctx, const ccx_dec_mid_chain_desc* desc, void* stream);
+
 typedef struct ccx_dec_beam_desc {
   const void* logits; int64_t ld; int n_vocab;
   int G, beam_size, max_candidates;
```

Result: faster. 1872 (median of 6 runs) (+2.3%).
